# Glaciohound/Chimera-ST

Hardware: AMD Instinct MI355X
Metric: train utterances/sec, MuST-C EN-DE s2t_transformer_m, 1/2/4/8 MI355X (higher is better)
Workload: dtype bf16

## Files before the change

chimera-st_amd/csrc/elementwise.hip:

```cpp
#include "cst_common.h"

namespace {

inline int ew_blocks(int64_t items) {
  int64_t b = cst_ceil_div(items, 256);
  return (int)(b < 1 ? 1 : (b > 4096 ? 4096 : b));
}

template <typename T>
__global__ void glu_fwd_kernel(const T* z, T* y, int64_t rows, int64_t C) {
  const int64_t cv = C / 8, total = rows * cv;
  for (int64_t i = (int64_t)blockIdx.x * blockDim.x + threadIdx.x; i < total; i += (int64_t)gridDim.x * blockDim.x) {
    const int64_t r = i / cv, c = (i % cv) * 8;
    float a[8], g[8], o[8];
    load8(z + r * 2 * C + c, a);
    load8(z + r * 2 * C + C + c, g);
#pragma unroll
    for (int e = 0; e < 8; ++e) o[e] = a[e] / (1.0f + __expf(-g[e]));
    store8(y + r * C + c, o);
  }
}

template <typename T>
__global__ void glu_bwd_kernel(const T* dy, const T* z, T* dz, int64_t rows, int64_t C) {
// ... 531 lines not shown
    hipLaunchKernelGGL(wn_apply_fwd_kernel<bf16_t>, dim3(blocks), dim3(256), 0, s, (const bf16_t*)v, (const bf16_t*)g, (bf16_t*)w, norm, (const float*)workspace, nch, R, (int)C);
  } else {
    hipLaunchKernelGGL((wn_partial_kernel<float, false>), dim3(nch), dim3(256), 0, s, (const float*)v, (const float*)nullptr, (float*)workspace, R, (int)C);
    hipLaunchKernelGGL(wn_apply_fwd_kernel<float>, dim3(blocks), dim3(256), 0, s, (const float*)v, (const float*)g, (float*)w, norm, (const float*)workspace, nch, R, (int)C);
  }
  return cst_check_launch("cst_weight_norm_fwd");
}

extern "C" int cst_weight_norm_bwd(const void* v, const void* g, const void* dw, const float* norm, void* dv, void* dg, void* workspace, int64_t R,
                                   int64_t C, int dtype, cst_stream stream) {
  CST_REQUIRE(v && g && dw && norm && dv && dg && workspace && R > 0, "cst_weight_norm_bwd: null tensor");
  CST_REQUIRE(C % 8 == 0 && C >= 8 && C <= 256 && 256 % (C / 8) == 0, "cst_weight_norm_bwd: C = %lld", (long long)C);
  hipStream_t s = (hipStream_t)stream;
  CstProfScope prof(CST_K_ELEMENTWISE, s, 0.0, (double)R * C * cst_dtype_size(dtype) * 5);
  const int nch = (int)cst_ceil_div(R, WN_ROWS);
  const int blocks = (int)(cst_ceil_div(R * (C / 8), 256) < 1024 ? cst_ceil_div(R * (C / 8), 256) : 1024);
  if (dtype == CST_BF16) {
    hipLaunchKernelGGL((wn_partial_kernel<bf16_t, true>), dim3(nch), dim3(256), 0, s, (const bf16_t*)v, (const bf16_t*)dw, (float*)workspace, R, (int)C);
    hipLaunchKernelGGL(wn_apply_bwd_kernel<bf16_t>, dim3(blocks), dim3(256), 0, s, (const bf16_t*)v, (const bf16_t*)g, (const bf16_t*)dw, norm, (bf16_t*)dv, (bf16_t*)dg,
                       (const float*)workspace, nch, R, (int)C);
  } else {
    hipLaunchKernelGGL((wn_partial_kernel<float, true>), dim3(nch), dim3(256), 0, s, (const float*)v, (const float*)dw, (float*)workspace, R, (int)C);
    hipLaunchKernelGGL(wn_apply_bwd_kernel<float>, dim3(blocks), dim3(256), 0, s, (const float*)v, (const float*)g, (const float*)dw, norm, (float*)dv, (float*)dg,
                       (const float*)workspace, nch, R, (int)C);
  }
  return cst_check_launch("cst_weight_norm_bwd");
}

namespace {
template <typename T>
__device__ __forceinline__ void transpose_tile(const T* src, T* dst, int64_t R, int64_t C, int64_t r0, int64_t c0, T* tile) {
  constexpr int V = DT<T>::VEC, TS = 64, LDT = TS + V;
  constexpr int VPR = TS / V;
  for (int v = threadIdx.x; v < TS * VPR; v += 256) {
    const int r = v / VPR, cv = (v % VPR) * V;
    u32x4 x = {0, 0, 0, 0};
    if (r0 + r < R && c0 + cv < C) x = *reinterpret_cast<const u32x4*>(src + (r0 + r) * C + c0 + cv);
    *reinterpret_cast<u32x4*>(tile + r * LDT + cv) = x;
  }
  __syncthreads();
  for (int v = threadIdx.x; v < TS * VPR; v += 256) {
    const int c = v / VPR, rv = (v % VPR) * V;
    if (c0 + c < C && r0 + rv < R) {
      T out[V];
#pragma unroll
      for (int e = 0; e < V; ++e) out[e] = tile[(rv + e) * LDT + c];
      *reinterpret_cast<u32x4*>(dst + (c0 + c) * R + r0 + rv) = *reinterpret_cast<const u32x4*>(out);
    }
  }
}

template <typename T>
__global__ __launch_bounds__(256) void transpose2d_kernel(const T* src, T* dst, int64_t R, int64_t C) {
  __shared__ __attribute__((aligned(16))) T tile[64 * (64 + DT<T>::VEC)];
  transpose_tile<T>(src, dst, R, C, (int64_t)blockIdx.y * 64, (int64_t)blockIdx.x * 64, tile);
}

template <typename T>
__global__ __launch_bounds__(256) void transpose2d_multi_kernel(const cst_transpose_item* items, int n) {
  __shared__ __attribute__((aligned(16))) T tile[64 * (64 + DT<T>::VEC)];
  const int64_t b = blockIdx.x;
  int lo = 0, hi = n - 1;
  while (lo < hi) {
    const int mid = (lo + hi + 1) >> 1;
    if (items[mid].tile0 <= b) lo = mid; else hi = mid - 1;
  }
  const cst_transpose_item it = items[lo];
  const int64_t t = b - it.tile0, tx = (it.C + 63) / 64;
  transpose_tile<T>((const T*)it.src, (T*)it.dst, it.R, it.C, (t / tx) * 64, (t % tx) * 64, tile);
}
}

extern "C" int cst_transpose2d_multi(const cst_transpose_item* items_dev, int n, int64_t total_tiles, int dtype, cst_stream stream) {
  CST_REQUIRE(items_dev && n > 0 && total_tiles > 0 && total_tiles < (1ll << 31), "cst_transpose2d_multi: bad table");
  CST_REQUIRE(dtype == CST_F32 || dtype == CST_BF16, "cst_transpose2d_multi: bad dtype");
  hipStream_t s = (hipStream_t)stream;
  CstProfScope prof(CST_K_ELEMENTWISE, s, 0.0, 2.0 * (double)total_tiles * 4096 * cst_dtype_size(dtype));
  if (dtype == CST_BF16) hipLaunchKernelGGL(transpose2d_multi_kernel<bf16_t>, dim3((unsigned)total_tiles), dim3(256), 0, s, items_dev, n);
  else hipLaunchKernelGGL(transpose2d_multi_kernel<float>, dim3((unsigned)total_tiles), dim3(256), 0, s, items_dev, n);
  return cst_check_launch("cst_transpose2d_multi");
}

namespace {
struct ReduceTable { cst_reduce_item it[CST_REDUCE_MAX_ITEMS]; int n; };

__global__ __launch_bounds__(1024) void reduce_multi_kernel(ReduceTable t) {
  __shared__ float ra[64][65];
  const int b = blockIdx.x;
  int lo = 0, hi = t.n - 1;
  while (lo < hi) {
    const int mid = (lo + hi + 1) >> 1;
    if (t.it[mid].block0 <= b) lo = mid; else hi = mid - 1;
  }
  const cst_reduce_item& it = t.it[lo];
  const int64_t blk = b - it.block0;
  if (it.order == 0) {
    const int64_t i0 = (blk * 1024 + threadIdx.x) * 8;
    if (i0 >= it.L) return;
    const float* src = it.src + i0;
    float v[8] = {0.0f, 0.0f, 0.0f, 0.0f, 0.0f, 0.0f, 0.0f, 0.0f};
    int sp = 0;
    for (; sp + 4 <= it.P; sp += 4) {
      f32x4 a[4][2];
#pragma unroll
      for (int u = 0; u < 4; ++u) {
        a[u][0] = *reinterpret_cast<const f32x4*>(src + (int64_t)(sp + u) * it.stride);
        a[u][1] = *reinterpret_cast<const f32x4*>(src + (int64_t)(sp + u) * it.stride + 4);
      }
#pragma unroll
      for (int u = 0; u < 4; ++u)
#pragma unroll
        for (int e = 0; e < 4; ++e) { v[e] += a[u][0][e]; v[4 + e] += a[u][1][e]; }
    }
    for (; sp < it.P; ++sp) {
      const f32x4 a0 = *reinterpret_cast<const f32x4*>(src + (int64_t)sp * it.stride), a1 = *reinterpret_cast<const f32x4*>(src + (int64_t)sp * it.stride + 4);
#pragma unroll
      for (int e = 0; e < 4; ++e) { v[e] += a0[e]; v[4 + e] += a1[e]; }
    }
    if (it.dst_dtype == CST_BF16) store8((bf16_t*)it.dst + i0, v);
    else store8((float*)it.dst + i0, v);
    return;
  }
  const int cl = threadIdx.x & 15, g = threadIdx.x >> 4;
  const int64_t c = blk * 64 + cl * 4;
  f32x4 a = {0.0f, 0.0f, 0.0f, 0.0f};
  if (c < it.L) {
    const float* src = it.src + c;
    int i = g;
    for (; i + 192 < it.P; i += 256) {
      const f32x4 v0 = *reinterpret_cast<const f32x4*>(src + (int64_t)i * it.stride), v1 = *reinterpret_cast<const f32x4*>(src + (int64_t)(i + 64) * it.stride);
      const f32x4 v2 = *reinterpret_cast<const f32x4*>(src + (int64_t)(i + 128) * it.stride), v3 = *reinterpret_cast<const f32x4*>(src + (int64_t)(i + 192) * it.stride);
#pragma unroll
      for (int e = 0; e < 4; ++e) a[e] = (((a[e] + v0[e]) + v1[e]) + v2[e]) + v3[e];
    }
    for (; i < it.P; i += 64) {
      const f32x4 v = *reinterpret_cast<const f32x4*>(src + (int64_t)i * it.stride);
#pragma unroll
      for (int e = 0; e < 4; ++e) a[e] += v[e];
    }
  }
#pragma unroll
  for (int e = 0; e < 4; ++e) ra[g][cl * 4 + e] = a[e];
  __syncthreads();
  if (threadIdx.x < 64) {
    const int64_t cc = blk * 64 + threadIdx.x;
    if (cc < it.L) {
      float t = ra[0][threadIdx.x];
#pragma unroll 8
      for (int k = 1; k < 64; ++k) t += ra[k][threadIdx.x];
      if (it.dst_dtype == CST_BF16) DT<bf16_t>::st((bf16_t*)it.dst + cc, t);
      else ((float*)it.dst)[cc] = t;
    }
  }
}
}

extern "C" int cst_reduce_multi(const cst_reduce_item* items, int n, cst_stream stream) {
  CST_REQUIRE(items && n > 0 && n <= CST_REDUCE_MAX_ITEMS, "cst_reduce_multi: 1..%d items per call", CST_REDUCE_MAX_ITEMS);
  ReduceTable t;
  int64_t blocks = 0;
  double bytes = 0.0;
  for (int i = 0; i < n; ++i) {
    const cst_reduce_item& it = items[i];
    CST_REQUIRE(it.src && it.dst && it.L > 0 && it.L % 8 == 0 && it.P > 0 && it.stride % 4 == 0 && ((uintptr_t)it.src % 16) == 0 && ((uintptr_t)it.dst % 16) == 0,
                "cst_reduce_multi: item %d: L, stride, alignment", i);
    CST_REQUIRE((it.dst_dtype == CST_F32 || it.dst_dtype == CST_BF16) && (it.order == 0 || it.order == 1), "cst_reduce_multi: item %d: bad dst_dtype / order", i);
// ... 25 lines not shown
```

chimera-st_amd/csrc/gemm.hip:

```cpp
#include "gemm_common.h"
#include <vector>
#include <stdlib.h>
#include <string.h>
#include <type_traits>

namespace {
using namespace cstg;

template <int BM_, int BN_, int WM_, int WN_, int KV_ = 8>
struct Cfg {
  static constexpr int BM = BM_, BN = BN_, WM = WM_, WN = WN_, NT = 64 * WM_ * WN_, TM = BM_ / WM_ / 32, TN = BN_ / WN_ / 32;
  static constexpr int KV = KV_;
  static_assert(BM_ <= GEMM_MAX_BM && GEMM_MAX_BM % BM_ == 0, "conv0.hip (cst_conv_row_limits) sizes live frames from GEMM_MAX_BM");
};
using CfgSmall = Cfg<128, 128, 2, 2>;
using CfgSkinny = Cfg<64, 64, 2, 2>;
using CfgNarrowN = Cfg<128, 64, 2, 2>;
using CfgNarrowM = Cfg<64, 128, 2, 2>;
using CfgLarge = Cfg<256, 256, 4, 4>;

template <typename T, bool A_KMAJOR, bool B_KMAJOR, bool SEG, typename C, bool CS = false>
__global__ __launch_bounds__(C::NT) void gemm_kernel(GemmParams p) {
  constexpr int BM = C::BM, BN = C::BN, NTHREADS = C::NT, TM = C::TM, TN = C::TN;
  constexpr int VEC = DT<T>::VEC;
  constexpr int KV = C::KV, BK = KV * VEC;
  constexpr int LDK = BK + VEC;
  constexpr int LDMA = sizeof(T) == 2 ? BM + 32 : BM + VEC;
  constexpr int LDMB = sizeof(T) == 2 ? BN + 32 : BN + VEC;
  constexpr int A_ELEMS = A_KMAJOR ? BM * LDK : BK * LDMA;
  constexpr int B_ELEMS = B_KMAJOR ? BN * LDK : BK * LDMB;
  constexpr int MVA = BM / VEC, MVB = BN / VEC;
  constexpr int NVA = BM * KV / NTHREADS, NVB = BN * KV / NTHREADS;
  extern __shared__ __attribute__((aligned(16))) char smem_raw[];
  T* smem = reinterpret_cast<T*>(smem_raw);
  constexpr int STAGE = A_ELEMS + B_ELEMS;

  const int tid = threadIdx.x, lane = tid & 63, wave = tid >> 6;
  const int wm = wave / C::WN, wn = wave % C::WN;

  const int ntiles = p.tiles_m * p.tiles_n;
  int tm, tn, z;
  if (p.split_order) {
    const int total = ntiles * p.splits, L = (int)blockIdx.x + (int)gridDim.x * (int)blockIdx.z;
    const int q = total / 8, r = total % 8, xcd = L % 8, loc = L / 8;
    const int item = (xcd < r ? xcd * (q + 1) : r * (q + 1) + (xcd - r) * q) + loc;
    z = item / ntiles;
    const int t = item % ntiles;
    tm = t / p.tiles_n;
    tn = t % p.tiles_n;
  } else {
    int id = blockIdx.x;
    {
      const int q = ntiles / 8, r = ntiles % 8, xcd = id % 8, loc = id / 8;
      id = (xcd < r ? xcd * (q + 1) : r * (q + 1) + (xcd - r) * q) + loc;
    }
    constexpr int GROUP_M = 8;
    const int per_group = GROUP_M * p.tiles_n;
    const int grp = id / per_group, rem = id % per_group;
    const int gm0 = grp * GROUP_M;
    const int gsz = (p.tiles_m - gm0 < GROUP_M) ? (p.tiles_m - gm0) : GROUP_M;
    tm = gm0 + rem % gsz;
    tn = rem / gsz;
    z = blockIdx.z;
  }
  const int64_t m0 = (int64_t)tm * BM, n0 = (int64_t)tn * BN;

  const int split = z % p.splits;
  const int64_t bidx = z / p.splits;
  const int64_t b0 = bidx / p.batch1, b1 = bidx % p.batch1;
  const T* A = (const T*)p.A + b0 * p.sa0 + b1 * p.sa1;
  const T* B = (const T*)p.B + b0 * p.sb0 + b1 * p.sb1;
  const int64_t cofs = b0 * p.sc0 + b1 * p.sc1;
  const int64_t bofs = b0 * p.sbias0 + b1 * p.sbias1;

  int ktiles = (int)((p.K + BK - 1) / BK);
  const int kfull = (int)(p.K / BK);
  if (p.k_len) {
    typedef const __attribute__((address_space(4))) int32_t* cptr_t;
    const int kl = ((cptr_t)p.k_len)[b0];
    const int live = kl <= 0 ? 0 : (kl + BK - 1) / BK;
    ktiles = live < ktiles ? live : ktiles;
  }
  const int per = (ktiles + p.splits - 1) / p.splits;
  const int kt0 = split * per;
  const int kt1 = (kt0 + per < ktiles) ? kt0 + per : ktiles;

  u32x4 ra[NVA], rb[NVB];
  const T* pa[NVA];
  const T* pb[NVB];
  int ka[NVA], kb[NVB];
  int aq[NVA], ar[NVA], bq[NVB], br[NVB];
#pragma unroll
  for (int i = 0; i < NVA; ++i) {
    const int v = tid + NTHREADS * i;
    if (A_KMAJOR) {
      int64_t row = m0 + v / KV;
      row = row < p.M ? row : p.M - 1;
      ka[i] = kt0 * BK + (v % KV) * VEC;
      if (SEG && p.a_seg) { aq[i] = ka[i] / (int)p.a_seg; ar[i] = ka[i] % (int)p.a_seg; pa[i] = A + row * p.lda; }
      else { aq[i] = 0; ar[i] = 0; pa[i] = A + row * p.lda + ka[i]; }
    } else {
      int64_t m = m0 + (int64_t)(v % MVA) * VEC;
      m = m < p.M ? m : p.M - VEC;
      ka[i] = kt0 * BK + v / MVA;
      aq[i] = 0; ar[i] = 0;
      pa[i] = A + (int64_t)ka[i] * p.lda + segaddr(m, p.a_seg, p.a_seg_stride);
    }
  }
#pragma unroll
  for (int i = 0; i < NVB; ++i) {
    const int v = tid + NTHREADS * i;
    if (B_KMAJOR) {
      int64_t row = n0 + v / KV;
      row = row < p.N ? row : p.N - 1;
      kb[i] = kt0 * BK + (v % KV) * VEC;
      if (SEG && p.b_seg) { bq[i] = kb[i] / (int)p.b_seg; br[i] = kb[i] % (int)p.b_seg; pb[i] = B + row * p.ldb; }
      else { bq[i] = 0; br[i] = 0; pb[i] = B + row * p.ldb + kb[i]; }
    } else {
      int64_t n = n0 + (int64_t)(v % MVB) * VEC;
      n = n < p.N ? n : p.N - VEC;
      kb[i] = kt0 * BK + v / MVB;
      bq[i] = 0; br[i] = 0;
      pb[i] = B + (int64_t)kb[i] * p.ldb + segaddr(n, p.b_seg, p.b_seg_stride);
    }
  }
  const int64_t step_a = A_KMAJOR ? (int64_t)BK : (int64_t)BK * p.lda;
  const int64_t step_b = B_KMAJOR ? (int64_t)BK : (int64_t)BK * p.ldb;

  auto load_tile = [&](auto tail_tag) {
    constexpr bool TAIL = decltype(tail_tag)::value;
    const u32x4 zero = {0, 0, 0, 0};
#pragma unroll
    for (int i = 0; i < NVA; ++i) {
      const T* qa = pa[i];
      if (SEG && A_KMAJOR && p.a_seg) qa = pa[i] + (int64_t)aq[i] * p.a_seg_stride + ar[i];
      if (TAIL) {
        const bool oka = ka[i] < p.K;
        const u32x4 va = *reinterpret_cast<const u32x4*>(oka ? qa : A);
        ra[i] = oka ? va : zero;
      } else {
        ra[i] = *reinterpret_cast<const u32x4*>(qa);
      }
      ka[i] += BK;
      if (SEG && A_KMAJOR && p.a_seg) { ar[i] += BK; while (ar[i] >= (int)p.a_seg) { ar[i] -= (int)p.a_seg; ++aq[i]; } }
      else pa[i] += step_a;
    }
#pragma unroll
    for (int i = 0; i < NVB; ++i) {
      const T* qb = pb[i];
      if (SEG && B_KMAJOR && p.b_seg) qb = pb[i] + (int64_t)bq[i] * p.b_seg_stride + br[i];
      if (TAIL) {
        const bool okb = kb[i] < p.K;
        const u32x4 vb = *reinterpret_cast<const u32x4*>(okb ? qb : B);
        rb[i] = okb ? vb : zero;
      } else {
        rb[i] = *reinterpret_cast<const u32x4*>(qb);
      }
      kb[i] += BK;
      if (SEG && B_KMAJOR && p.b_seg) { br[i] += BK; while (br[i] >= (int)p.b_seg) { br[i] -= (int)p.b_seg; ++bq[i]; } }
      else pb[i] += step_b;
    }
  };
  auto load_any = [&](int kt) {
    if (kt < kfull) load_tile(std::false_type{});
    else load_tile(std::true_type{});
  };
  static_assert(!CS || (!A_KMAJOR && NTHREADS % MVA == 0), "a thread must stage the same columns of an mn-major A in every vector");
  const bool do_cs = CS && tn == 0;
  float cs[VEC];
#pragma unroll
  for (int e = 0; e < VEC; ++e) cs[e] = 0.0f;
  auto store_tile = [&](int buf) {
#pragma unroll
    for (int i = 0; i < NVA; ++i) {
      const int v = tid + NTHREADS * i;
      T* da = smem + buf * STAGE + (A_KMAJOR ? (v / KV) * LDK + (v % KV) * VEC : (v / MVA) * LDMA + (v % MVA) * VEC);
      *reinterpret_cast<u32x4*>(da) = ra[i];
      if (CS && do_cs) {
        if (sizeof(T) == 2) {
#pragma unroll
          for (int e = 0; e < 4; ++e) {
            cs[2 * e] += __uint_as_float(ra[i][e] << 16);
            cs[2 * e + 1] += __uint_as_float(ra[i][e] & 0xffff0000u);
          }
        } else {
#pragma unroll
          for (int e = 0; e < 4; ++e) cs[e] += __uint_as_float(ra[i][e]);
        }
      }
    }
#pragma unroll
    for (int i = 0; i < NVB; ++i) {
      const int v = tid + NTHREADS * i;
      T* db = smem + buf * STAGE + A_ELEMS + (B_KMAJOR ? (v / KV) * LDK + (v % KV) * VEC : (v / MVB) * LDMB + (v % MVB) * VEC);
      *reinterpret_cast<u32x4*>(db) = rb[i];
    }
  };

  f32x16 acc[TM][TN];
#pragma unroll
  for (int i = 0; i < TM; ++i)
#pragma unroll
    for (int j = 0; j < TN; ++j)
#pragma unroll
      for (int r = 0; r < 16; ++r) acc[i][j][r] = 0.0f;

  constexpr int KLIST_MAX = 1000;
  __shared__ int klist[KLIST_MAX];
  __shared__ int klist_n;
  const bool kskip = !SEG && BK == 64 && p.k_live != nullptr && per <= KLIST_MAX;
  int nk = kt1 > kt0 ? kt1 - kt0 : 0;
  if (kskip) {
    if (wave == 0) {
      int total = 0;
      for (int base = 0; base < ktiles; base += 64) {
        const int kt = base + lane;
        total += __builtin_popcountll(__builtin_amdgcn_ballot_w64(kt < ktiles && p.k_live[kt] == p.k_epoch));
      }
      const int lo = (int)(((int64_t)total * split) / p.splits), hi = (int)(((int64_t)total * (split + 1)) / p.splits);
      int seen = 0, n = 0;
      for (int base = 0; base < ktiles && seen < hi; base += 64) {
        const int kt = base + lane;
        const bool live = kt < ktiles && p.k_live[kt] == p.k_epoch;
        const uint64_t m = __builtin_amdgcn_ballot_w64(live);
        const int idx = seen + __builtin_popcountll(m & ((1ull << lane) - 1ull));
        if (live && idx >= lo && idx < hi) klist[idx - lo] = kt;
        seen += __builtin_popcountll(m);
      }
      n = hi - lo;
      if (lane == 0) klist_n = n;
    }
    __syncthreads();
    nk = klist_n;
  }
  if (p.m_live) {
    typedef const __attribute__((address_space(4))) uint32_t* cptr_t;
    cptr_t ml = (cptr_t)p.m_live;
    const int t0 = (int)(m0 >> 6), t1 = (int)((((m0 + BM < p.M) ? m0 + BM : p.M) + 63) >> 6);
    bool live = false;
    for (int t = t0; t < t1; ++t) live |= ml[t] == p.m_epoch;
    if (!live) nk = 0;
  }
  if (p.m_len) {
    typedef const __attribute__((address_space(4))) int32_t* cptr_t;
    if (m0 >= (int64_t)((cptr_t)p.m_len)[b0]) nk = 0;
  }
  int pos = kt0;
  auto fetch = [&](int kt) {
    const int d = kt - pos;
    if (d) {
#pragma unroll
      for (int i = 0; i < NVA; ++i) { pa[i] += (int64_t)d * step_a; ka[i] += d * BK; }
#pragma unroll
      for (int i = 0; i < NVB; ++i) { pb[i] += (int64_t)d * step_b; kb[i] += d * BK; }
    }
    load_any(kt);
    pos = kt + 1;
  };
  auto tile_at = [&](int it) { return kskip ? klist[it] : kt0 + it; };

  if (nk > 0) {
    fetch(tile_at(0));
    store_tile(0);
  }
  __syncthreads();
  int cur = 0;
  const int lrow = lane & 31, lk = 8 * (lane >> 5);
  constexpr int WROWS = TM * 32, WCOLS = TN * 32;
  for (int it = 0; it < nk; ++it) {
    const bool more = it + 1 < nk;
    if (more) fetch(tile_at(it + 1));
    const T* sa = smem + cur * STAGE;
    const T* sb = sa + A_ELEMS;
#pragma unroll
    for (int kk = 0; kk < BK; kk += 16) {
      Frag<T> fa[TM], fb[TN];
#pragma unroll
      for (int i = 0; i < TM; ++i) {
        if (A_KMAJOR) frag_load_contig(fa[i], sa + (wm * WROWS + i * 32 + lrow) * LDK + kk + lk);
        else frag_load_tr(fa[i], sa, LDMA, wm * WROWS + i * 32, kk + lk, kk + lk + 4, lane);
      }
#pragma unroll
      for (int j = 0; j < TN; ++j) {
        if (B_KMAJOR) frag_load_contig(fb[j], sb + (wn * WCOLS + j * 32 + lrow) * LDK + kk + lk);
        else frag_load_tr(fb[j], sb, LDMB, wn * WCOLS + j * 32, kk + lk, kk + lk + 4, lane);
      }
#pragma unroll
      for (int i = 0; i < TM; ++i)
#pragma unroll
        for (int j = 0; j < TN; ++j) mma16(acc[i][j], fa[i], fb[j]);
    }
    if (more) store_tile(cur ^ 1);
    __syncthreads();
    cur ^= 1;
  }

  if (CS && do_cs) {
    float* red = reinterpret_cast<float*>(smem_raw);
#pragma unroll
    for (int e = 0; e < VEC; ++e) red[(tid / MVA) * BM + (tid % MVA) * VEC + e] = cs[e];
    __syncthreads();
    if (tid < BM && m0 + tid < p.M) {
      float tot = 0.0f;
      for (int r = 0; r < NTHREADS / MVA; ++r) tot += red[r * BM + tid];
      if (p.splits > 1) p.colsum_ws[((int64_t)bidx * p.splits + split) * p.M + m0 + tid] = tot;
      else DT<T>::st((T*)p.colsum + bidx * p.M + m0 + tid, tot);
    }
  }

  constexpr int LDC = BN + 4;
  constexpr int VPR = BN / 8;
  constexpr int NPASS = BM / 64;
  constexpr int ITERS = 64 * VPR / NTHREADS;
  float* stage = reinterpret_cast<float*>(smem_raw);
  float* wsp = p.splits > 1 ? p.ws + ((int64_t)z) * p.M * p.N : nullptr;
  const bool ws_vec = (p.N % 4) == 0;
#pragma unroll
  for (int ps = 0; ps < NPASS; ++ps) {
    __syncthreads();
#pragma unroll
    for (int i = 0; i < TM; ++i) {
      const int trow = wm * WROWS + i * 32;
      if (trow / 64 == ps) {
#pragma unroll
        for (int j = 0; j < TN; ++j)
#pragma unroll
          for (int r = 0; r < 16; ++r)
            stage[(trow - 64 * ps + acc_row(r, lane)) * LDC + wn * WCOLS + j * 32 + lrow] = acc[i][j][r];
      }
    }
    __syncthreads();
#pragma unroll 2
    for (int it = 0; it < ITERS; ++it) {
      const int v = tid + NTHREADS * it;
      const int rl = v / VPR, cl = (v % VPR) * 8;
      const int64_t row = m0 + 64 * ps + rl, col = n0 + cl;
      if (row >= p.M || col >= p.N) continue;
      float x[8];
      {
        const f32x4 a = *reinterpret_cast<const f32x4*>(stage + rl * LDC + cl);
        const f32x4 b = *reinterpret_cast<const f32x4*>(stage + rl * LDC + cl + 4);
        x[0] = a[0]; x[1] = a[1]; x[2] = a[2]; x[3] = a[3]; x[4] = b[0]; x[5] = b[1]; x[6] = b[2]; x[7] = b[3];
      }
      const bool full = col + 8 <= p.N;
      if (wsp) {
        if (full && ws_vec) store8(wsp + row * p.N + col, x);
        else
          for (int e = 0; e < 8 && col + e < p.N; ++e) wsp[row * p.N + col + e] = x[e];
      } else if (full && p.vec_epi) {
        epilogue_store8<T>(p, cofs, bofs, row, col, x);
      } else {
        for (int e = 0; e < 8 && col + e < p.N; ++e) epilogue_store<T>(p, cofs, bofs, row, col + e, x[e]);
      }
    }
  }
}

template <int N>
__device__ __forceinline__ void wait_vmcnt() { asm volatile("s_waitcnt vmcnt(%0)" ::"n"(N) : "memory"); }

template <typename T, bool A_KMAJOR, bool B_KMAJOR, typename C, int NS>
__global__ __launch_bounds__(C::NT) void gemm_glds_kernel(GemmParams p) {
  constexpr int BM = C::BM, BN = C::BN, NTHREADS = C::NT, TM = C::TM, TN = C::TN, NWAVES = C::NT / 64;
  constexpr int ES = sizeof(T), VEC = DT<T>::VEC, BK = 128 / ES;
  constexpr int A_BYTES = A_KMAJOR ? BM * 128 : BK * BM * ES;
  constexpr int B_BYTES = B_KMAJOR ? BN * 128 : BK * BN * ES;
  constexpr int STAGE_BYTES = A_BYTES + B_BYTES;
  constexpr int GA = A_BYTES / 1024 / NWAVES, GB = B_BYTES / 1024 / NWAVES;
  extern __shared__ __attribute__((aligned(16))) char smem_raw[];

  const int tid = threadIdx.x, lane = tid & 63, wave = tid >> 6;
  const int wm = wave / C::WN, wn = wave % C::WN;
  const int ntiles = p.tiles_m * p.tiles_n;
  int id = blockIdx.x;
  {
    const int q = ntiles / 8, r = ntiles % 8, xcd = id % 8, loc = id / 8;
    id = (xcd < r ? xcd * (q + 1) : r * (q + 1) + (xcd - r) * q) + loc;
  }
  constexpr int GROUP_M = 8;
  int tm, tn;
  {
    const int per_group = GROUP_M * p.tiles_n;
    const int grp = id / per_group, rem = id % per_group;
    const int gm0 = grp * GROUP_M;
    const int gsz = (p.tiles_m - gm0 < GROUP_M) ? (p.tiles_m - gm0) : GROUP_M;
    tm = gm0 + rem % gsz;
    tn = rem / gsz;
  }
  const int64_t m0 = (int64_t)tm * BM, n0 = (int64_t)tn * BN;
  const int z = blockIdx.z;
  const int split = z % p.splits;
  const int64_t bidx = z / p.splits;
  const int64_t b0 = bidx / p.batch1, b1 = bidx % p.batch1;
  const T* A = (const T*)p.A + b0 * p.sa0 + b1 * p.sa1;
  const T* B = (const T*)p.B + b0 * p.sb0 + b1 * p.sb1;
  const int64_t cofs = b0 * p.sc0 + b1 * p.sc1;
  const int64_t bofs = b0 * p.sbias0 + b1 * p.sbias1;
  const int ktiles = (int)((p.K + BK - 1) / BK);
  const int kfull = (int)(p.K / BK);
  const int per = (ktiles + p.splits - 1) / p.splits;
  const int kt0 = split * per;
  const int kt1 = (kt0 + per < ktiles) ? kt0 + per : ktiles;
  int nt = kt1 - kt0;
  if (p.m_len) {
    typedef const __attribute__((address_space(4))) int32_t* cptr_t;
    if (m0 >= (int64_t)((cptr_t)p.m_len)[b0]) nt = 0;
  }

  const T* pa[GA];
  const T* pb[GB];
  int ka[GA], kb[GB];
#pragma unroll
  for (int i = 0; i < GA; ++i) {
    const int g = wave + NWAVES * i;
    if (A_KMAJOR) {
      const int r = 8 * g + (lane >> 3), c = (lane & 7) ^ ((r >> 1) & 7);
      int64_t row = m0 + r;
      row = row < p.M ? row : p.M - 1;
      ka[i] = kt0 * BK + c * VEC;
      pa[i] = A + row * p.lda + ka[i];
// ... 334 lines not shown
  p.tiles_m = (int)cst_ceil_div(M, C::BM);
  p.tiles_n = (int)cst_ceil_div(N, C::BN);
  p.split_order = (p.splits > 1 && nbatch == 1) ? 1 : 0;
  dim3 grid(p.tiles_m * p.tiles_n, 1, (unsigned)(nbatch * p.splits));
  if constexpr (!AK && !BK_ && !SEG && C::NT <= 256) {
    if (p.colsum) {
      static bool attr_cs = false;
      if (!attr_cs) {
        (void)hipFuncSetAttribute(reinterpret_cast<const void*>(&gemm_kernel<T, AK, BK_, SEG, C, true>), hipFuncAttributeMaxDynamicSharedMemorySize, 160 * 1024 - 4096);
        attr_cs = true;
      }
      hipLaunchKernelGGL((gemm_kernel<T, AK, BK_, SEG, C, true>), grid, dim3(C::NT), lds, s, p);
      return cst_check_launch("cst_gemm");
    }
  }
  if (p.colsum) { cst_set_error("cst_gemm: internal: column sums requested from a configuration that does not build them"); return CST_ERR_UNSUPPORTED; }
  hipLaunchKernelGGL((gemm_kernel<T, AK, BK_, SEG, C>), grid, dim3(C::NT), lds, s, p);
  return cst_check_launch("cst_gemm");
}

template <typename T, bool AK, bool BK_, typename C, int NS>
int launch_glds(GemmParams p, int64_t M, int64_t N, int64_t nbatch, hipStream_t s) {
  constexpr int ES = sizeof(T), BKc = 128 / ES;
  constexpr int A_BYTES = AK ? C::BM * 128 : BKc * C::BM * ES, B_BYTES = BK_ ? C::BN * 128 : BKc * C::BN * ES;
  size_t lds = (size_t)NS * (A_BYTES + B_BYTES);
  const size_t stage_bytes = (size_t)64 * (C::BN + 4) * sizeof(float);
  if (lds < stage_bytes) lds = stage_bytes;
  static bool attr_set = false;
  if (!attr_set) {
    (void)hipFuncSetAttribute(reinterpret_cast<const void*>(&gemm_glds_kernel<T, AK, BK_, C, NS>), hipFuncAttributeMaxDynamicSharedMemorySize, 160 * 1024);
    attr_set = true;
  }
  p.tiles_m = (int)cst_ceil_div(M, C::BM);
  p.tiles_n = (int)cst_ceil_div(N, C::BN);
  dim3 grid(p.tiles_m * p.tiles_n, 1, (unsigned)(nbatch * p.splits));
  hipLaunchKernelGGL((gemm_glds_kernel<T, AK, BK_, C, NS>), grid, dim3(C::NT), lds, s, p);
  return cst_check_launch("cst_gemm");
}


struct GemmSwitches {
  bool no_klive;
  int group_m;
  bool no_narrow;
  bool no_4w;
  bool experiment;
  const char* force_cfg;
};

GemmSwitches gemm_switches() {
  static const GemmSwitches once = [] {
    GemmSwitches w;
    w.no_klive = getenv("CST_GEMM_NO_KLIVE") != nullptr;
    const char* gm = getenv("CST_GEMM8P_GROUP_M");
    w.group_m = gm && atoi(gm) > 0 ? atoi(gm) : 4;
    w.no_narrow = getenv("CST_GEMM_NO_NARROW") != nullptr;
    w.no_4w = getenv("CST_GEMM_NO_4W") != nullptr;
    w.experiment = getenv("CST_GEMM_EXPERIMENT") != nullptr;
    w.force_cfg = nullptr;
    return w;
  }();
  GemmSwitches w = once;
  if (w.experiment) {
    const char* f = getenv("CST_GEMM_FORCE_CFG");
    w.force_cfg = f && *f ? f : nullptr;
  }
  return w;
}

enum class Family { Reg, Dma, Persistent8, FourWave };
enum class Tile { Small, Large, Skinny, NarrowN, NarrowM, Big4, Big4N, Unknown };
enum class Colsum { None, Fused, Separate };
using CfgBig4 = Cfg<256, 256, 2, 2>;
using CfgBig4N = Cfg<256, 192, 2, 2>;

struct GemmRoute {
  Family family;
  Tile tile;
  bool bf16, ak, bk;
  bool seg;
  int stages;
  int splits;
  Colsum colsum;
};

struct TileDims { int bm, bn, nt; };
template <typename C> constexpr TileDims dims_of() { return {C::BM, C::BN, C::NT}; }
constexpr TileDims kTileDims[] = {dims_of<CfgSmall>(),   dims_of<CfgLarge>(), dims_of<CfgSkinny>(), dims_of<CfgNarrowN>(),
                                  dims_of<CfgNarrowM>(), dims_of<CfgBig4>(),  dims_of<CfgBig4N>(),  {0, 0, 0}};

bool use_large(const cst_gemm_desc* d, bool seg, int splits) {
  if (seg) return false;
  const int64_t tiles = cst_ceil_div(d->M, 256) * cst_ceil_div(d->N, 256) * d->batch0 * d->batch1 * splits;
  return d->M >= 256 && d->N >= 256 && tiles >= 200;
}

int choose_splits(const cst_gemm_desc* d) {
  if (d->split_k > 1) return d->split_k;
  if (d->split_k == 0 || d->split_k == 1) return 1;
  const int bk = d->dtype == CST_BF16 ? 64 : 32;
  const int64_t ktiles = cst_ceil_div(d->K, bk);
  const int64_t nb = d->batch0 * d->batch1;
  if (d->M >= 256 && d->N >= 256) {
    const int64_t tl = cst_ceil_div(d->M, 256) * cst_ceil_div(d->N, 256) * nb;
    if (tl >= 200) return 1;
    int64_t s = 256 / tl;
    if (s > ktiles / 16) s = ktiles / 16;
    if (s > 32) s = 32;
    if (s >= 1 && tl * s >= 200) return (int)s;
  }
  const int64_t tiles = cst_ceil_div(d->M, 128) * cst_ceil_div(d->N, 128) * nb;
  if (tiles >= 256 || ktiles < 16) return 1;
  const int64_t cap = ktiles / 8 < 32 ? ktiles / 8 : 32;
  int64_t s1 = 256 / tiles, s2 = 512 / tiles;
  if (s1 > cap) s1 = cap;
  if (s2 > cap) s2 = cap;
  if (s1 < 1) s1 = 1;
  if (s2 < 1) s2 = 1;
  const int64_t s = (2.0 / (double)s2 < 0.9 / (double)s1) ? s2 : s1;
  return (int)s;
}

struct Forced { const char* name; bool kk; Family family; Tile tile; int stages; };
const Forced kForced[] = {
    {"small", false, Family::Reg, Tile::Small, 0},     {"narrowm", false, Family::Reg, Tile::NarrowM, 0},
    {"narrown", false, Family::Reg, Tile::NarrowN, 0}, {"skinny", false, Family::Reg, Tile::Skinny, 0},
    {"large", false, Family::Reg, Tile::Large, 0},     {"big4r", false, Family::Reg, Tile::Big4, 0},
    {"skinny4", true, Family::Dma, Tile::Skinny, 4},   {"skinny2", true, Family::Dma, Tile::Skinny, 2},
    {"small2", true, Family::Dma, Tile::Small, 2},     {"small3", true, Family::Dma, Tile::Small, 3},
    {"big4", true, Family::Dma, Tile::Big4, 2},        {"big4n", true, Family::Dma, Tile::Big4N, 2},
    {"big4r", true, Family::Reg, Tile::Big4, 0},       {"large", true, Family::Reg, Tile::Large, 0},
    {"8p", true, Family::Persistent8, Tile::Large, 0}, {"4w", true, Family::FourWave, Tile::Big4N, 0},
};

GemmRoute gemm_route(const cst_gemm_desc* d, const GemmParams& p, const GemmSwitches& sw) {
  GemmRoute r;
  r.bf16 = d->dtype == CST_BF16;
  r.ak = d->a_kmajor != 0;
  r.bk = d->b_kmajor != 0;
  r.seg = (r.ak && d->a_seg) || (r.bk && d->b_seg);
  r.stages = 2;
  r.splits = choose_splits(d);
  const bool kk = r.ak && r.bk, mm = !r.ak && !r.bk;
  const bool large = use_large(d, r.seg, r.splits);
  const int64_t nbatch = d->batch0 * d->batch1;
  r.colsum = !d->colsum ? Colsum::None : (mm && !d->a_seg && !d->b_seg && !large) ? Colsum::Fused : Colsum::Separate;
  auto take = [&r](Family f, Tile t, int stages = 2) { r.family = f; r.tile = t; r.stages = stages; return r; };

  if (!sw.no_narrow && !r.seg && !large && kk && d->N <= 64 && d->M > 256) return take(Family::Dma, Tile::NarrowN);
  if (!sw.no_narrow && !r.seg && !large && mm && d->M <= 64 && d->N > 256) return take(Family::Reg, Tile::NarrowM);

  GemmParams q = p;
  q.splits = r.splits;
  const bool unsplit1 = !r.seg && nbatch == 1 && r.splits == 1;
  if (sw.force_cfg && r.bf16 && !r.seg && nbatch == 1 && (mm || (kk && r.splits == 1))) {
    for (const Forced& f : kForced) {
      if (f.kk != kk || strcmp(f.name, sw.force_cfg) != 0) continue;
      if (f.family == Family::Persistent8 && !cst_gemm8p_supported(q, r.ak, r.bk, nbatch)) break;
      if (f.family == Family::FourWave && !cst_gemm4w_supported(q, r.ak, r.bk, nbatch)) break;
      return take(f.family, f.tile, f.stages);
    }
    return take(Family::Reg, Tile::Unknown);
  }

  const bool mid8p = kk && unsplit1 && d->M >= 256 && d->N >= 256 && cst_ceil_div(d->M, 256) * cst_ceil_div(d->N, 256) >= 150;
  if (kk && unsplit1 && (d->M <= 256 || (!large && !mid8p && cst_ceil_div(d->M, 128) * cst_ceil_div(d->N, 128) < 256))) {
    const bool two_stage = d->M > 256 && cst_ceil_div(d->M, 64) * cst_ceil_div(d->N, 64) > 512;
    return take(Family::Dma, Tile::Skinny, two_stage ? 2 : 4);
  }
  if (r.bf16 && !r.seg && !d->colsum) {
    if (!sw.no_4w && cst_gemm4w_supported(q, r.ak, r.bk, nbatch)) return take(Family::FourWave, Tile::Big4N);
    if (r.ak && (!d->dact || (!d->resid && !d->aux_out)) && (large || mid8p) && cst_gemm8p_supported(q, r.ak, r.bk, nbatch))
      return take(Family::Persistent8, Tile::Large);
  }
  const Tile t = large ? Tile::Large : Tile::Small;
  if (r.seg) return take(Family::Reg, Tile::Small);
  return take(kk && !d->colsum ? Family::Dma : Family::Reg, t);
}

void route_text(const GemmRoute& r, char* out, int64_t n) {
  const TileDims t = kTileDims[(int)r.tile];
  const char* dt = r.bf16 ? "bf16" : "f32";
  const char a = r.ak ? 'k' : 'm', b = r.bk ? 'k' : 'm';
  switch (r.family) {
    case Family::Reg:
      snprintf(out, (size_t)n, "reg %s %c%c%s %dx%d nt%d%s split%d", dt, a, b, r.seg ? " seg" : "", t.bm, t.bn, t.nt,
               r.colsum == Colsum::Fused ? " colsum" : "", r.splits);
      break;
    case Family::Dma: snprintf(out, (size_t)n, "glds %s %c%c %dx%d nt%d ns%d split%d", dt, a, b, t.bm, t.bn, t.nt, r.stages, r.splits); break;
    case Family::Persistent8: snprintf(out, (size_t)n, "8p %c%c", a, b); break;
    case Family::FourWave: snprintf(out, (size_t)n, "4w"); break;
  }
}

}

extern "C" int64_t cst_colsum_workspace(int64_t rows, int64_t cols);
extern "C" int cst_colsum_typed(const void* x, int64_t ldx, void* out, void* workspace, int64_t rows, int64_t cols, int dtype, int out_dtype, cst_stream stream);
extern "C" int cst_colsum_typed_live(const void* x, int64_t ldx, void* out, void* workspace, int64_t rows, int64_t cols, int dtype, int out_dtype,
                                     const uint32_t* row_live, uint32_t epoch, cst_stream stream);

namespace {

int validate(const cst_gemm_desc* d) {
  CST_REQUIRE(d && d->A && d->B && d->C, "cst_gemm: null operand");
  CST_REQUIRE(d->dtype == CST_F32 || d->dtype == CST_BF16, "cst_gemm: bad dtype %d", d->dtype);
  CST_REQUIRE(d->c_dtype == d->dtype || d->c_dtype == CST_F32, "cst_gemm: c_dtype must be dtype or f32");
  CST_REQUIRE(d->M > 0 && d->N > 0 && d->K > 0, "cst_gemm: empty problem M=%lld N=%lld K=%lld", (long long)d->M,
              (long long)d->N, (long long)d->K);
  const int vec = d->dtype == CST_BF16 ? 8 : 4;
  if (d->a_kmajor) CST_REQUIRE(d->K % vec == 0 && d->lda % vec == 0, "cst_gemm: k-major A needs K,lda %% %d == 0 (K=%lld lda=%lld)", vec, (long long)d->K, (long long)d->lda);
  else CST_REQUIRE(d->M % vec == 0 && d->lda % vec == 0, "cst_gemm: mn-major A needs M,lda %% %d == 0 (M=%lld lda=%lld)", vec, (long long)d->M, (long long)d->lda);
  if (d->b_kmajor) CST_REQUIRE(d->K % vec == 0 && d->ldb % vec == 0, "cst_gemm: k-major B needs K,ldb %% %d == 0 (K=%lld ldb=%lld)", vec, (long long)d->K, (long long)d->ldb);
  else CST_REQUIRE(d->N % vec == 0 && d->ldb % vec == 0, "cst_gemm: mn-major B needs N,ldb %% %d == 0 (N=%lld ldb=%lld)", vec, (long long)d->N, (long long)d->ldb);
  CST_REQUIRE(d->a_seg % vec == 0 && d->b_seg % vec == 0 && d->a_seg_stride % vec == 0 && d->b_seg_stride % vec == 0,
              "cst_gemm: segment sizes must be multiples of %d", vec);
  CST_REQUIRE(((uintptr_t)d->A % 16 == 0) && ((uintptr_t)d->B % 16 == 0), "cst_gemm: A/B must be 16-byte aligned");
  CST_REQUIRE(d->sa0 % vec == 0 && d->sa1 % vec == 0 && d->sb0 % vec == 0 && d->sb1 % vec == 0, "cst_gemm: batch strides of A/B must be multiples of %d", vec);
  CST_REQUIRE(d->batch0 >= 1 && d->batch1 >= 1, "cst_gemm: batch counts must be >= 1");
  CST_REQUIRE(!d->dact || d->aux_in, "cst_gemm: dact needs aux_in");
  CST_REQUIRE(d->drop_p >= 0.0f && d->drop_p < 1.0f, "cst_gemm: drop_p must be in [0, 1)");
  CST_REQUIRE(d->drop_p == 0.0f || d->batch0 * d->batch1 == 1, "cst_gemm: fused dropout needs an unbatched problem");
  CST_REQUIRE(!d->colsum || (!d->a_kmajor && !d->a_seg), "cst_gemm: colsum needs an mn-major, unsegmented A");
  return CST_OK;
}

GemmParams fill_params(const cst_gemm_desc* d, const GemmSwitches& sw) {
  GemmParams p;
  p.M = d->M; p.N = d->N; p.K = d->K;
  p.A = d->A; p.lda = d->lda; p.a_seg = d->a_seg; p.a_seg_stride = d->a_seg_stride;
  p.B = d->B; p.ldb = d->ldb; p.b_seg = d->b_seg; p.b_seg_stride = d->b_seg_stride;
  p.C = d->C; p.ldc = d->ldc;
  p.bias = d->bias; p.bias_mode = d->bias ? d->bias_mode : CST_BIAS_NONE; p.sbias0 = d->sbias0; p.sbias1 = d->sbias1;
  p.act = d->act;
  p.aux_out = d->aux_out; p.ld_aux_out = d->ld_aux_out;
  p.dact = d->dact; p.aux_in = d->aux_in; p.ld_aux_in = d->ld_aux_in;
  p.resid = d->resid; p.ld_resid = d->ld_resid;
  p.alpha = d->alpha;
  p.drop_thr = d->drop_p > 0.0f ? cst_drop_thr16(d->drop_p) : 0u;
  p.drop_key = d->drop_key;
  p.drop_scale = d->drop_p > 0.0f ? 1.0f / (1.0f - d->drop_p) : 1.0f;
  p.drop_row0 = 0;
  p.batch1 = d->batch1;
  p.sa0 = d->sa0; p.sa1 = d->sa1; p.sb0 = d->sb0; p.sb1 = d->sb1; p.sc0 = d->sc0; p.sc1 = d->sc1;
  p.c_f32 = (d->c_dtype == CST_F32 && d->dtype != CST_F32) ? 1 : 0;
  {
    auto al16 = [](const void* q) { return q == nullptr || ((uintptr_t)q % 16) == 0; };
    bool ok = d->ldc % 8 == 0 && d->sc0 % 8 == 0 && d->sc1 % 8 == 0 && al16(d->C) && al16(d->bias) && al16(d->aux_out) && al16(d->aux_in) && al16(d->resid);
    if (d->bias && d->bias_mode == CST_BIAS_COL) ok = ok && d->sbias0 % 8 == 0 && d->sbias1 % 8 == 0;
    if (d->aux_out) ok = ok && d->ld_aux_out % 8 == 0;
    if (d->aux_in) ok = ok && d->ld_aux_in % 8 == 0;
    if (d->resid) ok = ok && d->ld_resid % 8 == 0;
    if (d->drop_p > 0.0f) ok = ok && (d->N % 2 == 0);
    p.vec_epi = ok ? 1 : 0;
  }
  p.tiles_m = p.tiles_n = 0;
  p.split_order = 0;
  p.sched = nullptr;
  p.gperm_full = 0;
  p.mrot = 0;
  p.k_live = sw.no_klive ? nullptr : d->k_live;
  p.k_epoch = d->k_epoch;
  p.m_live = sw.no_klive ? nullptr : d->m_live;
  p.m_epoch = d->m_epoch;
  p.k_len = sw.no_klive ? nullptr : d->k_len;
  p.m_len = sw.no_klive ? nullptr : d->m_len;
  p.group_m = sw.group_m;
  p.splits = 1;
  p.ws = nullptr;
  p.colsum = nullptr;
  p.colsum_ws = nullptr;
  return p;
}

int64_t route_workspace(const cst_gemm_desc* d, const GemmRoute& r) {
  const int64_t s = r.splits, nb = d->batch0 * d->batch1;
  int64_t bytes = s > 1 ? s * d->M * d->N * nb * (int64_t)sizeof(float) : 0;
  if (r.colsum == Colsum::Fused) bytes += s > 1 ? s * d->M * nb * (int64_t)sizeof(float) : 0;
  else if (r.colsum == Colsum::Separate) bytes += cst_colsum_workspace(d->K, d->M);
  return bytes;
}

int take_route(const cst_gemm_desc* d, const GemmSwitches& sw, GemmParams& p, GemmRoute& r) {
  r = gemm_route(d, p, sw);
  const int64_t nbatch = d->batch0 * d->batch1;
  CST_REQUIRE(r.colsum != Colsum::Separate || (nbatch == 1 && d->M % 8 == 0 && d->lda % 8 == 0),
              "cst_gemm: colsum of this configuration runs as a separate column sum: unbatched, M and lda multiples of 8");
  CST_REQUIRE(cst_ceil_div(d->M, 128) * cst_ceil_div(d->N, 128) < (1ll << 31) && nbatch * r.splits < 65536, "cst_gemm: grid too large");
  p.splits = r.splits;
  p.colsum = r.colsum == Colsum::Fused ? d->colsum : nullptr;
#ifdef CST_TRACE
  if (p.splits == 1 && d->workspace) p.ws = (float*)d->workspace;
#endif
  const int64_t need = route_workspace(d, r);
  if (need > 0 && (!d->workspace || d->workspace_bytes < need)) {
    if (r.splits > 1) cst_set_error("cst_gemm: split_k=%d needs %lld workspace bytes, got %lld", r.splits, (long long)need, (long long)d->workspace_bytes);
    else cst_set_error("cst_gemm: colsum needs %lld workspace bytes, got %lld", (long long)need, (long long)d->workspace_bytes);
    return CST_ERR_WORKSPACE;
  }
  if (r.splits > 1) {
    p.ws = (float*)d->workspace;
    p.colsum_ws = p.ws + (int64_t)r.splits * d->M * d->N * nbatch;
  }
  return CST_OK;
}

template <typename W>
bool read_back(hipStream_t s, const W* dev, int64_t n, std::vector<W>& host) {
  host.resize((size_t)n);
  return hipStreamSynchronize(s) == hipSuccess && hipMemcpy(host.data(), dev, sizeof(W) * n, hipMemcpyDeviceToHost) == hipSuccess;
}

struct Work { double flops, bytes; };
Work credited_work(const cst_gemm_desc* d, const GemmParams& p, hipStream_t s) {
  double frac = 1.0;
  if (cst_prof_is_on()) {
    std::vector<uint32_t> st;
    std::vector<int32_t> len;
    const int64_t mtiles = cst_ceil_div(d->M, 256);
    if (p.k_live && read_back(s, p.k_live, cst_ceil_div(d->K, 64), st)) {
      int64_t live = 0;
      for (uint32_t v : st) live += v == p.k_epoch;
      frac *= (double)live / (double)st.size();
    }
    if (p.k_len && read_back(s, p.k_len, d->batch0, len)) {
      double sum = 0.0;
      for (int32_t v : len) sum += (double)(v < 0 ? 0 : (v < d->K ? v : d->K));
      frac *= sum / ((double)d->batch0 * (double)d->K);
    }
    if (p.m_len && read_back(s, p.m_len, d->batch0, len)) {
      double live = 0.0;
      for (int32_t v : len) {
        const int64_t t = v <= 0 ? 0 : cst_ceil_div((int64_t)v, 256);
        live += (double)(t < mtiles ? t : mtiles);
      }
      frac *= live / ((double)d->batch0 * (double)mtiles);
    }
    if (p.m_live && read_back(s, p.m_live, cst_ceil_div(d->M, 64), st)) {
      const int64_t nt = (int64_t)st.size();
      int64_t live = 0;
      for (int64_t t = 0; t < mtiles; ++t) {
        bool l = false;
        for (int64_t i = 4 * t; i < 4 * t + 4 && i < nt; ++i) l |= st[i] == p.m_epoch;
        live += l;
      }
      frac *= (double)live / (double)mtiles;
    }
  }
  const double nbatch = (double)(d->batch0 * d->batch1), esz = (double)cst_dtype_size(d->dtype);
  return {2.0 * (double)d->M * (double)d->N * (double)d->K * nbatch * frac,
          ((double)d->M * d->K + (double)d->N * d->K) * esz * nbatch * frac + (double)d->M * d->N * cst_dtype_size(d->c_dtype) * nbatch};
}

int unlaunchable(const GemmRoute& r, const GemmSwitches& sw) {
  if (r.tile == Tile::Unknown) {
    cst_set_error("cst_gemm: unknown CST_GEMM_FORCE_CFG %s", sw.force_cfg ? sw.force_cfg : "");
    return CST_ERR_BAD_ARG;
  }
  if (r.family == Family::Reg && r.colsum == Colsum::Fused && kTileDims[(int)r.tile].nt > 256) {
    cst_set_error("cst_gemm: internal: column sums requested from a configuration that does not build them");
    return CST_ERR_UNSUPPORTED;
  }
  return CST_OK;
}

template <typename T, bool SEG, typename C>
int launch_reg(const GemmRoute& r, const GemmParams& p, int64_t nbatch, hipStream_t s) {
  return r.ak ? (r.bk ? launch<T, true, true, SEG, C>(p, p.M, p.N, nbatch, s) : launch<T, true, false, SEG, C>(p, p.M, p.N, nbatch, s))
// ... 10 lines not shown
    case arm(Family::Persistent8, Tile::Large): return cst_gemm8p_launch(p, r.ak, r.bk, nbatch, s);
    case arm(Family::FourWave, Tile::Big4N): return cst_gemm4w_launch(p, s);
    case arm(Family::Reg, Tile::Small): return r.seg ? launch_reg<T, true, CfgSmall>(r, p, nbatch, s) : launch_reg<T, false, CfgSmall>(r, p, nbatch, s);
    case arm(Family::Reg, Tile::Large): return launch_reg<T, false, CfgLarge>(r, p, nbatch, s);
    case arm(Family::Reg, Tile::NarrowM): return launch<T, false, false, false, CfgNarrowM>(p, M, N, nbatch, s);
    case arm(Family::Dma, Tile::Small, 2): return launch_glds<T, true, true, CfgSmall, 2>(p, M, N, nbatch, s);
    case arm(Family::Dma, Tile::Large, 2): return launch_glds<T, true, true, CfgLarge, 2>(p, M, N, nbatch, s);
    case arm(Family::Dma, Tile::NarrowN, 2): return launch_glds<T, true, true, CfgNarrowN, 2>(p, M, N, nbatch, s);
    case arm(Family::Dma, Tile::Skinny, 2): return launch_glds<T, true, true, CfgSkinny, 2>(p, M, N, nbatch, s);
    case arm(Family::Dma, Tile::Skinny, 4): return launch_glds<T, true, true, CfgSkinny, 4>(p, M, N, nbatch, s);
    case arm(Family::Reg, Tile::NarrowN): if constexpr (HOOK) return launch<T, false, false, false, CfgNarrowN>(p, M, N, nbatch, s); break;
    case arm(Family::Reg, Tile::Skinny): if constexpr (HOOK) return launch<T, false, false, false, CfgSkinny>(p, M, N, nbatch, s); break;
    case arm(Family::Reg, Tile::Big4):
      if constexpr (HOOK) return r.ak ? launch<T, true, true, false, CfgBig4>(p, M, N, nbatch, s) : launch<T, false, false, false, CfgBig4>(p, M, N, nbatch, s);
      break;
    case arm(Family::Dma, Tile::Small, 3): if constexpr (HOOK) return launch_glds<T, true, true, CfgSmall, 3>(p, M, N, nbatch, s); break;
    case arm(Family::Dma, Tile::Big4, 2): if constexpr (HOOK) return launch_glds<T, true, true, CfgBig4, 2>(p, M, N, nbatch, s); break;
    case arm(Family::Dma, Tile::Big4N, 2): if constexpr (HOOK) return launch_glds<T, true, true, CfgBig4N, 2>(p, M, N, nbatch, s); break;
    default: break;
  }
  const int rc = unlaunchable(r, sw);
  if (rc == CST_OK) cst_set_error("cst_gemm: internal: a route without a launch arm");
  return rc == CST_OK ? CST_ERR_UNSUPPORTED : rc;
}

int finish(const cst_gemm_desc* d, const GemmRoute& r, const GemmParams& p, cst_stream stream) {
  const int64_t nbatch = d->batch0 * d->batch1;
  if (p.splits > 1 && d->defer_reduce) {
    CST_REQUIRE((nbatch == 1 || !d->colsum) && d->alpha == 1.0f && !d->bias && !d->act && !d->dact && !d->aux_out && !d->resid && d->drop_p == 0.0f && d->ldc == d->N &&
                    d->N % 8 == 0 && r.colsum != Colsum::Separate,
                "cst_gemm: defer_reduce needs a plain epilogue and a dense C (batched: no colsum; the slabs are [batch][split][M][N])");
    return CST_OK;
  }
  int rc = CST_OK;
  if (p.splits > 1) {
    const int64_t total = d->M * d->N;
    const int64_t work = (p.vec_epi && d->N % 8 == 0) ? total / 8 : total;
    int blocks = (int)(cst_ceil_div(work, 256) < 2048 ? cst_ceil_div(work, 256) : 2048);
    dim3 grid(blocks, (unsigned)nbatch);
    if (d->dtype == CST_BF16) hipLaunchKernelGGL(splitk_reduce_kernel<bf16_t>, grid, dim3(256), 0, (hipStream_t)stream, p);
    else hipLaunchKernelGGL(splitk_reduce_kernel<float>, grid, dim3(256), 0, (hipStream_t)stream, p);
    rc = cst_check_launch("cst_gemm split-k reduce");
  }
  if (rc == CST_OK && r.colsum == Colsum::Separate) {
    void* cws = (char*)d->workspace + (p.splits > 1 ? (int64_t)p.splits * d->M * d->N * (int64_t)sizeof(float) : 0);
    rc = p.k_live ? cst_colsum_typed_live(d->A, d->lda, d->colsum, cws, d->K, d->M, d->dtype, d->dtype, p.k_live, p.k_epoch, stream)
                  : cst_colsum_typed(d->A, d->lda, d->colsum, cws, d->K, d->M, d->dtype, d->dtype, stream);
  }
  return rc;
}

int gemm_one(const cst_gemm_desc* d, cst_stream stream) {
  int rc = validate(d);
  if (rc != CST_OK) return rc;
  const GemmSwitches sw = gemm_switches();
  GemmParams p = fill_params(d, sw);
  GemmRoute r;
  if ((rc = take_route(d, sw, p, r)) != CST_OK) return rc;
  hipStream_t s = (hipStream_t)stream;
  const int64_t nbatch = d->batch0 * d->batch1;
  const Work w = credited_work(d, p, s);
  CstProfScope prof(CST_K_GEMM, s, w.flops, w.bytes);
  rc = r.bf16 ? launch_route<bf16_t>(r, p, nbatch, s, sw) : launch_route<float>(r, p, nbatch, s, sw);
  if (cst_prof_is_on())
    prof.tag("M=%lld N=%lld K=%lld b=%lld a%c b%c split=%d%s%s%s%s%s%s%s", (long long)d->M, (long long)d->N, (long long)d->K, (long long)nbatch, r.ak ? 'k' : 'm',
             r.bk ? 'k' : 'm', p.splits, d->bias ? " bias" : "", d->act ? " act" : "", d->aux_out ? " aux_out" : "", d->dact ? " dact" : "",
             d->resid ? " resid" : "", d->drop_p > 0 ? " drop" : "", (d->k_live || d->m_live || d->k_len || d->m_len) ? " live" : "");
  return rc != CST_OK ? rc : finish(d, r, p, stream);
}

GemmRoute query_route(const cst_gemm_desc* d) {
  const GemmSwitches sw = gemm_switches();
  return gemm_route(d, fill_params(d, sw), sw);
}

}

extern "C" int cst_gemm_splits(const cst_gemm_desc* d) { return d ? query_route(d).splits : 0; }

extern "C" int cst_gemm_colsum_is_fused(const cst_gemm_desc* d) { return d && query_route(d).colsum == Colsum::Fused ? 1 : 0; }

extern "C" int64_t cst_gemm_workspace(const cst_gemm_desc* d) { return route_workspace(d, query_route(d)); }

extern "C" int cst_gemm_route(const cst_gemm_desc* d, char* out, int64_t out_bytes) {
  if (out && out_bytes > 0) out[0] = 0;
  int rc = validate(d);
  if (rc != CST_OK) return rc;
  CST_REQUIRE(out && out_bytes > 0, "cst_gemm_route: no room for the text");
  const GemmSwitches sw = gemm_switches();
  GemmParams p = fill_params(d, sw);
  GemmRoute r;
  if ((rc = take_route(d, sw, p, r)) != CST_OK) return rc;
  if ((rc = unlaunchable(r, sw)) != CST_OK) return rc;
  route_text(r, out, out_bytes);
  return CST_OK;
}

extern "C" int cst_gemm(const cst_gemm_desc* d, cst_stream stream) { return gemm_one(d, stream); }
```

chimera-st_amd/csrc/gemm8p.hip:

```cpp
#include "gemm_common.h"
#include <atomic>
#include <cstdlib>
#include <mutex>
#include <type_traits>

namespace {
using namespace cstg;
using T = bf16_t;

constexpr int BM = 256, BN = 256, BK = 64, NTHREADS = 512;
static_assert(BM <= cstg::GEMM_MAX_BM && cstg::GEMM_MAX_BM % BM == 0, "conv0.hip (cst_conv_row_limits) sizes live frames from GEMM_MAX_BM");
constexpr int QB = 17408;
constexpr int GSTRIDE = 1088;
constexpr int KSTRIDE = 1024;
constexpr int BUFB = 4 * QB;
constexpr int LDS_BYTES = 2 * BUFB;
constexpr unsigned OOB = 0x80000000u;

template <int N>
__device__ __forceinline__ void wait_vm() { asm volatile("s_waitcnt vmcnt(%0)" ::"n"(N) : "memory"); }
template <int N>
__device__ __forceinline__ void wait_lgkm() { asm volatile("s_waitcnt lgkmcnt(%0)" ::"n"(N) : "memory"); }

__device__ __forceinline__ unsigned lds_off(const void* p) {
// ... 29 lines not shown
  const int wave = __builtin_amdgcn_readfirstlane(tid >> 6);
  const int wm = wave >> 2, wn = wave & 3;
  const int lrow = lane & 31, hi = lane >> 5;
  const int ntiles = p.tiles_m * p.tiles_n;
  const int total = p.nitems;
  const int ktiles = (int)((p.K + BK - 1) / BK);
  const int per = (ktiles + p.splits - 1) / p.splits;
  typedef const __attribute__((address_space(4))) GemmParams* kparg_t;
  kparg_t kp = (kparg_t)__builtin_amdgcn_kernarg_segment_ptr();

  const int ck = (lane & 7) ^ (((4 * wave) + (lane >> 4)) & 7);
  const int klm = 16 * (wave >> 2) + 4 * (lane >> 4) + (wave & 3);
  const int kla = AK ? ck * 8 : klm, klb = BKM ? ck * 8 : klm;
  const int pa = AK ? 8 * wave + (lane >> 3) : (lane & 15) * 8;
  const int pb = BKM ? 8 * wave + (lane >> 3) : (lane & 15) * 8;
  const unsigned step_a = AK ? (unsigned)(BK * 2) : (unsigned)(BK * p.lda * 2);
  const unsigned step_b = BKM ? (unsigned)(BK * 2) : (unsigned)(BK * p.ldb * 2);
  constexpr bool EXF = MODE == 2;
  const bool fast_epi = MODE != 0 || (!p.c_f32 && p.splits == 1 && p.vec_epi && (p.N % 8) == 0 && p.bias_mode != CST_BIAS_ROW &&
                                (p.bias_mode == CST_BIAS_NONE || p.alpha == 1.0f));
  const bool bias_in_acc = fast_epi && p.bias_mode == CST_BIAS_COL;
  char* const bias_lds = smem + 2 * BUFB;

  __amdgpu_buffer_rsrc_t ra, rb;
  unsigned va0 = 0, vb0 = 0;
  int nt = 0, krem0 = 0, mrem = 0, nrem = 0;
  int hf = 0;
  unsigned lda2 = 0, ldb2 = 0;
  int64_t m0 = 0, n0 = 0, cofs = 0, bofs = 0;
  int zcur = 0;

  auto setup = [&](int v) {
    asm volatile("" : "+s"(kp));
    struct { int64_t M, N, K, lda, ldb, batch1, sa0, sa1, sb0, sb1, sc0, sc1, sbias0, sbias1; const void *A, *B, *bias; int splits, tiles_m, tiles_n; } p;
    p.M = kp->M; p.N = kp->N; p.K = kp->K; p.lda = kp->lda; p.ldb = kp->ldb; p.batch1 = kp->batch1;
    p.sa0 = kp->sa0; p.sa1 = kp->sa1; p.sb0 = kp->sb0; p.sb1 = kp->sb1; p.sc0 = kp->sc0; p.sc1 = kp->sc1;
    p.sbias0 = kp->sbias0; p.sbias1 = kp->sbias1; p.A = kp->A; p.B = kp->B; p.bias = kp->bias;
    p.splits = kp->splits; p.tiles_m = kp->tiles_m; p.tiles_n = kp->tiles_n;
    auto fdiv = [](int n, unsigned long long magic) { return (int)(((unsigned long long)(unsigned)n * magic) >> 40); };
    int half = -1, vt = v;
    if (v >= kp->half_from) {
      const int o = v - kp->half_from;
      half = o & 1;
      vt = kp->half_from + (o >> 1);
    }
    hf = half >= 0 ? 1 : 0;
    const int z = kp->nz > 1 ? fdiv(vt, kp->magic_ntiles) : 0;
    int id = vt - z * ntiles;
    {
      const int q = ntiles >> 3, r = ntiles & 7, xcd = id & 7, loc = id >> 3;
      id = (xcd < r ? xcd * (q + 1) : r * (q + 1) + (xcd - r) * q) + loc;
    }
    if (kp->mrot > 0) {
      int zr = z * kp->mrot;
      zr -= fdiv(zr, kp->magic_ntiles) * ntiles;
      id += zr;
      if (id >= ntiles) id -= ntiles;
    }
    const int GROUP_M = kp->group_m, per_group = kp->per_group, gshift = kp->group_shift;
    int grp = fdiv(id, kp->magic_per_group);
    const int rem = id - grp * per_group;
    if (kp->gperm_full > 0 && grp < kp->gperm_full) {
      const int q = kp->gperm_q, r = kp->gperm_r, big = (q + 1) * r;
      int col, row;
      if (grp < big) { col = fdiv(grp, kp->magic_gq1); row = grp - col * (q + 1); }
      else { const int t = grp - big, c = fdiv(t, kp->magic_gq); col = r + c; row = t - c * q; }
      grp = row * 8 + col;
    }
    const int gm0 = grp * GROUP_M;
    const int gsz = (p.tiles_m - gm0 < GROUP_M) ? (p.tiles_m - gm0) : GROUP_M;
    int tm, tn;
    if (gsz == GROUP_M && gshift >= 0) { tm = gm0 + (rem & (GROUP_M - 1)); tn = rem >> gshift; }
    else { tm = gm0 + rem % gsz; tn = rem / gsz; }
    m0 = (int64_t)tm * BM + (half == 1 ? 128 : 0);
    n0 = (int64_t)tn * BN;
    zcur = z;
    const int split = p.splits > 1 ? z % p.splits : 0;
    const int64_t bidx = p.splits > 1 ? z / p.splits : z;
    const int64_t b0 = p.batch1 > 1 ? bidx / p.batch1 : bidx, b1 = p.batch1 > 1 ? bidx % p.batch1 : 0;
    const T* A = (const T*)p.A + b0 * p.sa0 + b1 * p.sa1;
    const T* B = (const T*)p.B + b0 * p.sb0 + b1 * p.sb1;
    cofs = b0 * p.sc0 + b1 * p.sc1;
    bofs = b0 * p.sbias0 + b1 * p.sbias1;
    const int kt0 = split * per;
    const int kt1 = (kt0 + per < ktiles) ? kt0 + per : ktiles;
    nt = kt1 > kt0 ? kt1 - kt0 : 0;
    if (kp->m_live) {
      typedef const __attribute__((address_space(4))) uint32_t* cptr_t;
      cptr_t ml = (cptr_t)kp->m_live;
      const uint32_t ep = kp->m_epoch;
      const int t0 = (int)(m0 >> 6), tn = (int)((p.M + 63) >> 6);
      bool live = false;
#pragma unroll
      for (int i = 0; i < 4; ++i) live |= (i < 2 || !hf) && (t0 + i < tn) && ml[t0 + i < tn ? t0 + i : t0] == ep;
      if (!live) nt = 0;
    }
    if (kp->m_len) {
      typedef const __attribute__((address_space(4))) int32_t* iptr_t;
      if (m0 >= (int64_t)((iptr_t)kp->m_len)[b0]) nt = 0;
    }
    krem0 = (int)p.K - kt0 * BK;
    const T* abase = AK ? A + m0 * p.lda + (int64_t)kt0 * BK : A + (int64_t)kt0 * BK * p.lda + m0;
    const T* bbase = BKM ? B + n0 * p.ldb + (int64_t)kt0 * BK : B + (int64_t)kt0 * BK * p.ldb + n0;
    ra = __builtin_amdgcn_make_buffer_rsrc((void*)abase, (short)0, (int)OOB, 0x00020000);
    rb = __builtin_amdgcn_make_buffer_rsrc((void*)bbase, (short)0, (int)OOB, 0x00020000);
    if (bias_in_acc) {
      const int64_t left = p.N - n0;
      const __amdgpu_buffer_rsrc_t rbias = __builtin_amdgcn_make_buffer_rsrc((void*)((const T*)p.bias + bofs + n0), (short)0,
                                                                              (int)((left < 256 ? left : 256) * 2), 0x00020000);
      dma16(rbias, bias_lds, (unsigned)lane * 16);
    }
    lda2 = (unsigned)(p.lda * 2);
    ldb2 = (unsigned)(p.ldb * 2);
    mrem = (int)(p.M - m0 < BM ? p.M - m0 : BM);
    if (hf && mrem > 128) mrem = 128;
    if (mrem <= 0) { mrem = 0; nt = 0; }
    nrem = (int)(p.N - n0 < BN ? p.N - n0 : BN);
    va0 = AK ? (unsigned)pa * lda2 + (unsigned)kla * 2 : (unsigned)klm * lda2 + (unsigned)pa * 2;
    vb0 = BKM ? (unsigned)pb * ldb2 + (unsigned)klb * 2 : (unsigned)klm * ldb2 + (unsigned)pb * 2;
  };

  auto stage = [&](auto qc, auto bufc, int tau) {
    constexpr int Q = decltype(qc)::value, BUF = decltype(bufc)::value;
    constexpr bool IS_A = (Q & 1) != 0;
    constexpr int H = Q >> 1;
    constexpr bool KM = IS_A ? AK : BKM;
    constexpr int GS = KM ? KSTRIDE : GSTRIDE;
    const int krem = krem0 - tau * BK;
    const unsigned ld2 = IS_A ? lda2 : ldb2;
    const unsigned base = (IS_A ? va0 : vb0) + (unsigned)tau * (IS_A ? step_a : step_b) + (KM ? (unsigned)(H * 128) * ld2 : (unsigned)(H * 256));
    const int pos = (IS_A ? pa : pb) + H * 128;
    const int lim = IS_A ? mrem : nrem;
    char* dst = smem + BUF * BUFB + Q * QB + wave * GS;
#pragma unroll
    for (int j = 0; j < 2; ++j) {
      const unsigned v0 = base + (KM ? (unsigned)(64 * j) * ld2 : (unsigned)(32 * j) * ld2);
      const bool ok = ((IS_A ? kla : klb) + (KM ? 0 : 32 * j) < krem) && (pos + (KM ? 64 * j : 0) < lim);
      dma16(IS_A ? ra : rb, dst + j * 8 * GS, ok ? v0 : OOB);
    }
  };
  using I0 = std::integral_constant<int, 0>;
  using I1 = std::integral_constant<int, 1>;
  using I2 = std::integral_constant<int, 2>;
  using I3 = std::integral_constant<int, 3>;

  const int swr = (lrow >> 1) & 7;
  const int arow = (wm * 64 + lrow) * 128, brow = (wn * 32 + lrow) * 128;
  const int trl = ((lane & 15) >> 2) * GSTRIDE + hi * 512 + (16 * ((lane >> 4) & 1) + 4 * (lane & 3)) * 2;
  auto read_tr = [&](Frag<T>& f, const char* q) {
    const v4s_t x = __builtin_amdgcn_ds_read_tr16_b64_v4i16((v4s_t __attribute__((address_space(3)))*)(q));
    const v4s_t y = __builtin_amdgcn_ds_read_tr16_b64_v4i16((v4s_t __attribute__((address_space(3)))*)(q + 256));
    u16x8 t;
    t[0] = (unsigned short)x[0]; t[1] = (unsigned short)x[1]; t[2] = (unsigned short)x[2]; t[3] = (unsigned short)x[3];
    t[4] = (unsigned short)y[0]; t[5] = (unsigned short)y[1]; t[6] = (unsigned short)y[2]; t[7] = (unsigned short)y[3];
    f.v = __builtin_bit_cast(bf16x8, t);
  };
  auto read_a = [&](Frag<T>& f, const char* img, int i, int kk) {
    if (AK) f.v = *reinterpret_cast<const bf16x8*>(img + arow + i * 4096 + (((2 * kk + hi) ^ swr) << 4));
    else read_tr(f, img + trl + wm * 128 + i * 64 + kk * 4 * GSTRIDE);
  };
  auto read_b = [&](Frag<T>& f, const char* img, int kk) {
    if (BKM) f.v = *reinterpret_cast<const bf16x8*>(img + brow + (((2 * kk + hi) ^ swr) << 4));
    else read_tr(f, img + trl + wn * 64 + kk * 4 * GSTRIDE);
  };

  f32x16 acc[4][2];
  Frag<T> fa[2][4], fb0[4], fb1[4];

  auto mfma_quadrant = [&](auto hmc, auto hnc) {
    constexpr int HM = decltype(hmc)::value, HN = decltype(hnc)::value;
    __builtin_amdgcn_s_setprio(1);
#pragma unroll
    for (int kk = 0; kk < 4; ++kk)
#pragma unroll
      for (int i = 0; i < 2; ++i) mma16(acc[HM * 2 + i][HN], HN ? fb1[kk] : fb0[kk], fa[i][kk]);
    __builtin_amdgcn_s_setprio(0);
  };

  auto tile_body = [&](auto bufc, int t, int S, const bool half) {
    constexpr int BUF = decltype(bufc)::value;
    using BC = std::integral_constant<int, BUF>;
    using BN_ = std::integral_constant<int, BUF ^ 1>;
    const char* img = smem + BUF * BUFB;
    const int s0 = 7 + 4 * t;
#pragma unroll
    for (int kk = 0; kk < 4; ++kk) read_b(fb0[kk], img + 0 * QB, kk);
    __builtin_amdgcn_sched_barrier(0);
#pragma unroll
    for (int kk = 0; kk < 4; ++kk)
#pragma unroll
      for (int i = 0; i < 2; ++i) read_a(fa[i][kk], img + 1 * QB, i, kk);
    __builtin_amdgcn_sched_barrier(0);
    if (s0 < S) stage(I3{}, BN_{}, t + 1);
    wait_lgkm<AK ? 8 : 15>();
    __builtin_amdgcn_s_barrier();
    wait_lgkm<0>();
    __builtin_amdgcn_sched_barrier(0);
// ... 54 lines not shown
    const int S = 4 * nt;
    if (0 < S) stage(I0{}, I0{}, 0);
    if (1 < S) stage(I1{}, I0{}, 0);
    if (2 < S) stage(I2{}, I0{}, 0);
    if (3 < S) stage(I3{}, I0{}, 0);
  }
  claim_issue();
  claim_land();
#ifdef CST_TRACE
  long long* trace = (p.splits == 1 && p.ws) ? reinterpret_cast<long long*>(p.ws) + (int64_t)blockIdx.x * 64 : nullptr;
  int titem = 0;
#define CST_STAMP(k) do { if (trace && tid == 0 && titem < 8) trace[titem * 8 + (k)] = (long long)__builtin_readcyclecounter(); } while (0)
#else
#define CST_STAMP(k) do { } while (0)
#endif
  while (true) {
    CST_STAMP(0);
    const int64_t e_m0 = m0, e_n0 = n0, e_cofs = cofs, e_bofs = bofs;
    const int e_z = zcur, e_nt = nt;
    const bool e_hf = hf != 0;
    const int S = 4 * e_nt;
    if (4 < S) stage(I0{}, I1{}, 1);
    if (5 < S) stage(I1{}, I1{}, 1);
    if (6 < S) stage(I2{}, I1{}, 1);
    if (7 <= S) wait_vm<6>();
    else wait_vm<0>();
    __builtin_amdgcn_s_barrier();
    if (bias_in_acc) {
#pragma unroll
      for (int hn = 0; hn < 2; ++hn)
#pragma unroll
        for (int g = 0; g < 4; ++g) {
          const uint2 raw = *reinterpret_cast<const uint2*>(bias_lds + (hn * 128 + wn * 32 + 8 * g + 4 * hi) * 2);
          const float b0 = __uint_as_float(raw.x << 16), b1 = __uint_as_float(raw.x & 0xffff0000u);
          const float b2 = __uint_as_float(raw.y << 16), b3 = __uint_as_float(raw.y & 0xffff0000u);
#pragma unroll
          for (int i = 0; i < 4; ++i) {
            acc[i][hn][4 * g] = b0; acc[i][hn][4 * g + 1] = b1; acc[i][hn][4 * g + 2] = b2; acc[i][hn][4 * g + 3] = b3;
          }
        }
      wait_lgkm<0>();
    } else {
#pragma unroll
      for (int i = 0; i < 4; ++i)
#pragma unroll
        for (int j = 0; j < 2; ++j)
#pragma unroll
          for (int r = 0; r < 16; ++r) acc[i][j][r] = 0.0f;
    }
    if (wm == 1) __builtin_amdgcn_s_barrier();
    CST_STAMP(1);
    for (int t = 0; t < e_nt; t += 2) {
      tile_body(I0{}, t, S, e_hf);
      if (t + 1 < e_nt) tile_body(I1{}, t + 1, S, e_hf);
    }
    if (wm == 0) __builtin_amdgcn_s_barrier();
    CST_STAMP(2);

    {
      int item;
      asm volatile("ds_read_b32 %0, %1\n\ts_waitcnt lgkmcnt(0)" : "=v"(item) : "v"(slot_off + 4u * (unsigned)par) : "memory");
      v = __builtin_amdgcn_readfirstlane(p.sched ? item : v + (int)gridDim.x);
    }
    const bool has_next = v < total;
    if (has_next) {
      claim_issue();
      setup(v);
      CST_STAMP(5);
      const int Sn = 4 * nt;
      if (0 < Sn) stage(I0{}, I0{}, 0);
      if (1 < Sn) stage(I1{}, I0{}, 0);
      if (2 < Sn) stage(I2{}, I0{}, 0);
      if (3 < Sn) stage(I3{}, I0{}, 0);
      CST_STAMP(6);
    }

    CST_STAMP(3);
    asm volatile("" : "+s"(kp));
    GemmParams q;
    q.M = kp->M; q.N = kp->N; q.C = kp->C; q.ldc = kp->ldc; q.bias = kp->bias; q.bias_mode = kp->bias_mode; q.act = kp->act;
    q.aux_out = kp->aux_out; q.ld_aux_out = kp->ld_aux_out; q.dact = kp->dact; q.aux_in = kp->aux_in; q.ld_aux_in = kp->ld_aux_in;
    q.resid = kp->resid; q.ld_resid = kp->ld_resid; q.alpha = kp->alpha; q.splits = kp->splits; q.ws = kp->ws;
    q.c_f32 = kp->c_f32; q.vec_epi = kp->vec_epi; q.drop_thr = kp->drop_thr; q.drop_key = kp->drop_key; q.drop_scale = kp->drop_scale; q.drop_row0 = kp->drop_row0;
    if (fast_epi && e_nt == 0 && q.bias_mode == CST_BIAS_NONE && !q.resid) {
      if (has_next) claim_land();
      const u32x4 z4 = {0u, 0u, 0u, 0u};
      const int64_t col = e_n0 + (tid & 31) * 8;
      if (col < q.N) {
        T* const cb = (T*)q.C + e_cofs + col;
        T* const xb = q.aux_out ? (T*)q.aux_out + e_cofs + col : nullptr;
#pragma unroll 4
        for (int it = 0; it < (e_hf ? 8 : 16); ++it) {
          const int64_t row = e_m0 + (tid >> 5) + 16 * it;
          if (row < q.M) {
            __builtin_nontemporal_store(z4, reinterpret_cast<u32x4*>(cb + row * q.ldc));
            if (xb) __builtin_nontemporal_store(z4, reinterpret_cast<u32x4*>(xb + row * q.ld_aux_out));
          }
        }
      }
    } else if (fast_epi) {
      constexpr int ERS = 528;
      const T* exsrc = MODE == 1 ? nullptr : (q.dact ? (const T*)q.aux_in : (const T*)q.resid);
      const int64_t exld = q.dact ? q.ld_aux_in : q.ld_resid;
      const bool both = q.dact && q.resid;
      constexpr bool ex_fast = EXF;
      u32x4 exq[8];
      const T* ex_b = nullptr;
      if (ex_fast) {
        int64_t colc = e_n0 + (tid & 31) * 8;
        colc = colc < q.N ? colc : q.N - 8;
        ex_b = exsrc + e_cofs + colc;
#pragma unroll
        for (int it = 0; it < 8; ++it) {
          int64_t row = e_m0 + (tid >> 5) + 16 * it;
          row = row < q.M ? row : q.M - 1;
          exq[it] = __builtin_nontemporal_load(reinterpret_cast<const u32x4*>(ex_b + row * exld));
        }
      }
#pragma unroll
      for (int hm = 0; hm < 2; ++hm) {
        if (hm && e_hf) break;
        if (hm) __builtin_amdgcn_s_barrier();
#pragma unroll
        for (int i = 0; i < 2; ++i)
#pragma unroll
          for (int hn = 0; hn < 2; ++hn)
#pragma unroll
            for (int g = 0; g < 4; ++g) {
              typedef __bf16 bf16x4_t __attribute__((ext_vector_type(4)));
              bf16x4_t pk;
#pragma unroll
              for (int e = 0; e < 4; ++e) pk[e] = static_cast<__bf16>(acc[hm * 2 + i][hn][4 * g + e] * q.alpha);
              lds_write_b64(ebase_off + (wm * 64 + i * 32 + lrow) * ERS + (hn * 128 + wn * 32 + 8 * g + 4 * hi) * 2, __builtin_bit_cast(uint2, pk));
            }
        wait_lgkm<0>();
        __builtin_amdgcn_s_barrier();
        if (hm == 0 && has_next) claim_land();
        if (exsrc && !ex_fast) {
#pragma unroll 2
          for (int it = 0; it < 8; ++it) {
            const int vi = tid + NTHREADS * it;
            const int rl = vi >> 5, cl = (vi & 31) * 8;
            const int64_t row = e_m0 + hm * 128 + rl, col = e_n0 + cl;
            if (row >= q.M || col >= q.N) continue;
            const u32x4 exv = *reinterpret_cast<const u32x4*>(exsrc + e_cofs + row * exld + col);
            const u32x4 zraw = lds_read_b128(ebase_off + rl * ERS + cl * 2);
            wait_lgkm<0>();
            __builtin_amdgcn_sched_barrier(0);
            if (q.aux_out) *reinterpret_cast<u32x4*>((T*)q.aux_out + e_cofs + row * q.ld_aux_out + col) = zraw;
            float x[8];
#pragma unroll
            for (int e = 0; e < 4; ++e) {
              x[2 * e] = __uint_as_float(zraw[e] << 16);
              x[2 * e + 1] = __uint_as_float(zraw[e] & 0xffff0000u);
            }
            if (q.act == CST_ACT_RELU) {
#pragma unroll
              for (int e = 0; e < 8; ++e) x[e] = fmaxf(x[e], 0.0f);
            } else if (q.act == CST_ACT_GELU) {
#pragma unroll
              for (int e = 0; e < 8; ++e) x[e] = gelu_t<T>(x[e]);
            }
            if (q.drop_thr) cst_drop8(x, q.drop_key, (uint64_t)((row + q.drop_row0) * q.N + col), q.drop_thr, q.drop_scale);
            if (q.dact) {
#pragma unroll
              for (int e = 0; e < 4; ++e) {
// ... 157 lines not shown
          if (row >= q.M || col >= q.N) continue;
          float x[8];
          {
            const u32x4 ua = lds_read_b128(ebase_off + (rl * LDC + cl) * 4), ub = lds_read_b128(ebase_off + (rl * LDC + cl + 4) * 4);
            wait_lgkm<0>();
            __builtin_amdgcn_sched_barrier(0);
            const f32x4 a = __builtin_bit_cast(f32x4, ua), b = __builtin_bit_cast(f32x4, ub);
            x[0] = a[0]; x[1] = a[1]; x[2] = a[2]; x[3] = a[3]; x[4] = b[0]; x[5] = b[1]; x[6] = b[2]; x[7] = b[3];
          }
          const bool full = col + 8 <= q.N;
          if (wsp) {
            if (full && ws_vec) store8(wsp + row * q.N + col, x);
            else
              for (int e = 0; e < 8 && col + e < q.N; ++e) wsp[row * q.N + col + e] = x[e];
          } else if (full && q.vec_epi) {
            epilogue_store8<T>(q, e_cofs, e_bofs, row, col, x);
          } else {
            for (int e = 0; e < 8 && col + e < q.N; ++e) epilogue_store<T>(q, e_cofs, e_bofs, row, col + e, x[e]);
          }
        }
      }
    }
    CST_STAMP(4);
#ifdef CST_TRACE
    ++titem;
#endif
    if (!has_next) break;
    __builtin_amdgcn_s_barrier();
  }
  int* const sched_exit = p.sched;
  if (int* const sched = sched_exit; sched && tid == 0) {
    if (atomicAdd(sched + 8, 1) == (int)gridDim.x - 1) {
#pragma unroll
      for (int i = 0; i < 9; ++i) __hip_atomic_store(sched + i, 0, __ATOMIC_RELAXED, __HIP_MEMORY_SCOPE_AGENT);
    }
  }
}

int* sched_slot() {
  constexpr int SLOTS = 1024, MAXDEV = 64;
  static int* ring[MAXDEV] = {};
  static std::atomic<unsigned> next[MAXDEV];
  static std::mutex mu;
  int dev = 0;
  if (hipGetDevice(&dev) != hipSuccess || dev < 0 || dev >= MAXDEV) return nullptr;
  int* r = __atomic_load_n(&ring[dev], __ATOMIC_ACQUIRE);
  if (!r) {
    std::lock_guard<std::mutex> g(mu);
    r = ring[dev];
    if (!r) {
      void* q = nullptr;
      if (hipMalloc(&q, SLOTS * 64) != hipSuccess) return nullptr;
      if (hipMemset(q, 0, SLOTS * 64) != hipSuccess || hipDeviceSynchronize() != hipSuccess) return nullptr;
      r = (int*)q;
      __atomic_store_n(&ring[dev], r, __ATOMIC_RELEASE);
    }
  }
  return r + 16 * (next[dev].fetch_add(1, std::memory_order_relaxed) % SLOTS);
}

std::atomic<int> g_reserved_cus{[] { const char* e = getenv("CST_GEMM_RESERVE_CUS"); return e ? atoi(e) : 0; }()};

template <bool AK, bool BKM, int MODE>
int launch8p(GemmParams p, int64_t nbatch, hipStream_t s) {
  static bool attr_set = false;
  if (!attr_set) {
    (void)hipFuncSetAttribute(reinterpret_cast<const void*>(&gemm8p_kernel<AK, BKM, MODE>), hipFuncAttributeMaxDynamicSharedMemorySize, 160 * 1024);
    attr_set = true;
  }
  p.tiles_m = (int)cst_ceil_div(p.M, BM);
  p.tiles_n = (int)cst_ceil_div(p.N, BN);
  p.nz = (int)(nbatch * p.splits);
  const int64_t total = (int64_t)p.tiles_m * p.tiles_n * p.nz;
  {
    const int64_t ntl = (int64_t)p.tiles_m * p.tiles_n;
    p.per_group = p.group_m * p.tiles_n;
    if (total * ntl >= (1ll << 40) || total * (int64_t)p.per_group >= (1ll << 40)) { cst_set_error("cst_gemm (8-phase): too many work items"); return CST_ERR_BAD_ARG; }
    p.magic_ntiles = ((1ull << 40) / (unsigned long long)ntl) + 1ull;
    p.magic_per_group = ((1ull << 40) / (unsigned long long)p.per_group) + 1ull;
    p.group_shift = -1;
    for (int sft = 0; sft < 16; ++sft)
      if ((1 << sft) == p.group_m) p.group_shift = sft;
    const int gfull = p.tiles_m / p.group_m;
    p.gperm_full = (p.m_len && gfull >= 16) ? gfull : 0;
    p.mrot = (p.m_len && p.gperm_full == 0 && ntl >= 2) ? (int)(ntl / 8 > 0 ? ntl / 8 : 1) : 0;
    p.gperm_q = gfull / 8;
    p.gperm_r = gfull % 8;
    p.magic_gq = p.gperm_q > 0 ? ((1ull << 40) / (unsigned long long)p.gperm_q) + 1ull : 0ull;
    p.magic_gq1 = ((1ull << 40) / (unsigned long long)(p.gperm_q + 1)) + 1ull;
  }
  static const int ncu = [] {
    int dev = 0, n = 256;
    (void)hipGetDevice(&dev);
    (void)hipDeviceGetAttribute(&n, hipDeviceAttributeMultiprocessorCount, dev);
    return n > 0 ? n : 256;
  }();
  const int avail = ncu - g_reserved_cus.load(std::memory_order_relaxed) > 8 ? ncu - g_reserved_cus.load(std::memory_order_relaxed) : 8;
  const bool no_halves = getenv("CST_GEMM8P_NO_HALVES") != nullptr;
  int64_t nitems = total;
  p.half_from = 0x7fffffff;
  if (!no_halves && p.nz == 1 && total > avail) {
    const int64_t r = total % avail;
    if (r > 0 && 2 * r <= avail) {
      p.half_from = (int)(total - r);
      nitems = total + r;
    }
  }
  p.nitems = (int)nitems;
  dim3 grid((unsigned)(nitems < avail ? nitems : avail), 1, 1);
  static const bool static_walk = getenv("CST_GEMM8P_STATIC") != nullptr;
  hipStreamCaptureStatus cap = hipStreamCaptureStatusNone;
  const bool capturing = hipStreamIsCapturing(s, &cap) != hipSuccess || cap != hipStreamCaptureStatusNone;
  p.sched = (!static_walk && !capturing && nitems > avail && grid.x % 8 == 0) ? sched_slot() : nullptr;
  hipLaunchKernelGGL((gemm8p_kernel<AK, BKM, MODE>), grid, dim3(NTHREADS), LDS_BYTES + 1024 + 64, s, p);
  return cst_check_launch("cst_gemm (8-phase)");
}

}

extern "C" int cst_gemm_reserve_cus(int n) {
  const int old = g_reserved_cus.load();
  if (n >= 0) g_reserved_cus.store(n > 248 ? 248 : n);
  return old;
}

bool cst_gemm8p_supported(const cstg::GemmParams& p, bool ak, bool bk, int64_t nbatch) {
  (void)nbatch;
  if (p.a_seg || p.b_seg) return false;
  const int64_t lim = (int64_t)1 << 31;
  const int64_t ea = ak ? (256 * p.lda + p.K) * 2 : (p.K + 64) * p.lda * 2;
  const int64_t eb = bk ? (256 * p.ldb + p.K) * 2 : (p.K + 64) * p.ldb * 2;
  return ea < lim && eb < lim && p.lda > 0 && p.ldb > 0;
}

int cst_gemm8p_launch(cstg::GemmParams p, bool ak, bool bk, int64_t nbatch, hipStream_t s) {
  const bool fast = !p.c_f32 && p.splits == 1 && p.vec_epi && (p.N % 8) == 0 && p.bias_mode != CST_BIAS_ROW &&
                    (p.bias_mode == CST_BIAS_NONE || p.alpha == 1.0f);
  const bool exf = fast && !p.aux_out && ((p.dact != 0) != (p.resid != nullptr)) && (!p.dact || p.aux_in);
  const bool plainf = fast && !p.dact && !p.resid;
#define CST_8P_MODE(MODE)                                                                                          \
  (ak ? (bk ? launch8p<true, true, MODE>(p, nbatch, s) : launch8p<true, false, MODE>(p, nbatch, s))              \
      : (bk ? launch8p<false, true, MODE>(p, nbatch, s) : launch8p<false, false, MODE>(p, nbatch, s)))
  if (exf) return CST_8P_MODE(2);
  if (plainf) return CST_8P_MODE(1);
  return CST_8P_MODE(0);
#undef CST_8P_MODE
}
```

chimera-st_amd/csrc/gemm_common.h:

```cpp
#pragma once
#include "cst_common.h"

namespace cstg {

constexpr int GEMM_MAX_BM = 256;

struct GemmParams {
  int64_t M, N, K;
  const void* A; int64_t lda, a_seg, a_seg_stride;
  const void* B; int64_t ldb, b_seg, b_seg_stride;
  void* C; int64_t ldc;
  const void* bias; int bias_mode; int64_t sbias0, sbias1;
  int act;
  void* aux_out; int64_t ld_aux_out;
  int dact;
  const void* aux_in; int64_t ld_aux_in;
  const void* resid; int64_t ld_resid;
  float alpha;
  uint32_t drop_thr, drop_key; float drop_scale;
  int64_t drop_row0;
  int64_t batch1;
  int64_t sa0, sa1, sb0, sb1, sc0, sc1;
  int splits;
  float* ws;
  int c_f32;
  int vec_epi;
  int tiles_m, tiles_n;
  int nz;
  int half_from, nitems;
  int group_m;
  unsigned long long magic_ntiles, magic_per_group;
  int per_group, group_shift;
  int gperm_full, gperm_q, gperm_r;
  int mrot;
  unsigned long long magic_gq, magic_gq1;
  int split_order;
  int* sched;
  const uint32_t* m_live; uint32_t m_epoch;
  const int32_t* k_len;
  const int32_t* m_len;
  const uint32_t* k_live; uint32_t k_epoch;
  void* colsum;
  float* colsum_ws;
};

__device__ __forceinline__ int64_t segaddr(int64_t c, int64_t seg, int64_t seg_stride) {
  return seg ? (c / seg) * seg_stride + (c % seg) : c;
}

template <typename T>
__device__ __forceinline__ void epilogue_store(const GemmParams& p, int64_t cofs, int64_t bofs, int64_t row, int64_t col, float v) {
  v *= p.alpha;
  if (p.bias_mode == CST_BIAS_COL) v += DT<T>::ld((const T*)p.bias + bofs + col);
  else if (p.bias_mode == CST_BIAS_ROW) v += DT<T>::ld((const T*)p.bias + bofs + row);
  if (p.aux_out) DT<T>::st((T*)p.aux_out + cofs + row * p.ld_aux_out + col, v);
  v = act_t<T>(v, p.act);
  if (p.drop_thr) v *= cst_drop1(p.drop_key, (uint64_t)((row + p.drop_row0) * p.N + col), p.drop_thr, p.drop_scale);
  if (p.dact) v *= dact_t<T>(DT<T>::ld((const T*)p.aux_in + cofs + row * p.ld_aux_in + col), p.dact);
  if (p.resid) v += DT<T>::ld((const T*)p.resid + cofs + row * p.ld_resid + col);
  if (p.c_f32) ((float*)p.C)[cofs + row * p.ldc + col] = v;
  else DT<T>::st((T*)p.C + cofs + row * p.ldc + col, v);
}

template <typename T>
__device__ __forceinline__ void epilogue_store8(const GemmParams& p, int64_t cofs, int64_t bofs, int64_t row, int64_t col, float (&v)[8]) {
#pragma unroll
  for (int e = 0; e < 8; ++e) v[e] *= p.alpha;
  if (p.bias_mode == CST_BIAS_COL) {
    float b[8];
    load8((const T*)p.bias + bofs + col, b);
#pragma unroll
    for (int e = 0; e < 8; ++e) v[e] += b[e];
  } else if (p.bias_mode == CST_BIAS_ROW) {
    const float b = DT<T>::ld((const T*)p.bias + bofs + row);
#pragma unroll
    for (int e = 0; e < 8; ++e) v[e] += b;
  }
  if (p.aux_out) store8((T*)p.aux_out + cofs + row * p.ld_aux_out + col, v);
  if (p.act == CST_ACT_RELU) {
#pragma unroll
    for (int e = 0; e < 8; ++e) v[e] = fmaxf(v[e], 0.0f);
  } else if (p.act == CST_ACT_GELU) {
#pragma unroll
    for (int e = 0; e < 8; ++e) v[e] = gelu_t<T>(v[e]);
  }
  if (p.drop_thr) cst_drop8(v, p.drop_key, (uint64_t)((row + p.drop_row0) * p.N + col), p.drop_thr, p.drop_scale);
  if (p.dact) {
    float z[8];
    load8((const T*)p.aux_in + cofs + row * p.ld_aux_in + col, z);
#pragma unroll
    for (int e = 0; e < 8; ++e) v[e] *= dact_t<T>(z[e], p.dact);
  }
  if (p.resid) {
    float r[8];
    load8((const T*)p.resid + cofs + row * p.ld_resid + col, r);
#pragma unroll
    for (int e = 0; e < 8; ++e) v[e] += r[e];
  }
  if (p.c_f32) store8((float*)p.C + cofs + row * p.ldc + col, v);
  else store8((T*)p.C + cofs + row * p.ldc + col, v);
}

}

int cst_gemm8p_launch(cstg::GemmParams p, bool a_kmajor, bool b_kmajor, int64_t nbatch, hipStream_t s);
bool cst_gemm8p_supported(const cstg::GemmParams& p, bool a_kmajor, bool b_kmajor, int64_t nbatch);
int cst_gemm4w_launch(cstg::GemmParams p, hipStream_t s);
bool cst_gemm4w_supported(const cstg::GemmParams& p, bool a_kmajor, bool b_kmajor, int64_t nbatch);
```

chimera-st_amd/functional.py:

```python
import os as _os
import weakref as _weakref

import torch

from . import kernels as K
from . import lib as L

_ACT = {None: L.ACT_NONE, "none": L.ACT_NONE, "relu": L.ACT_RELU, "gelu": L.ACT_GELU}


def _flat2d(x):
    return x.reshape(-1, x.shape[-1]).contiguous()


def _vec(dtype):
    return 8 if dtype == torch.bfloat16 else 4


def _with_tiles(t, tiles):
    if t.is_contiguous():
        t._cst_live_tiles = (tiles[0], tiles[1], t.data_ptr(), t.numel(), t.shape[-1], t._version)
        if t._base is not None:
            t._base._cst_live_tiles = t._cst_live_tiles
    return t
# ... 700 lines not shown


def ln_gelu(u, ln_weight, ln_bias, conv_bias=None, eps=1e-5, row_limit=None):
    return _LnGeluFn.apply(u, ln_weight, ln_bias, conv_bias, eps, row_limit)


def _padded_base(t, L, C):
    if t.dim() == 3 and t.stride(2) == 1 and t.stride(1) == C and t.stride(0) == (L + 2) * C and t.storage_offset() >= C:
        return torch.as_strided(t, (t.shape[0], L + 2, C), t.stride(), t.storage_offset() - C)
    return None


class _Conv1dCLFn(torch.autograd.Function):

    @staticmethod
    def forward(ctx, x, w_cl, bias, k, stride, pad, act, prev_z, grad_is_dz, nz_out=None, nz_in=None, unread_ok=False):
        if _os.environ.get("CST_NO_MLEN"):
            nz_in = None
            fwd_len = None
        else:
            fwd_len = nz_out if (bias is None or unread_ok) else None
        ctx.nz_out = nz_out
        ctx.nz_in = nz_in
        B, Lin, Cin = x.shape
        Cout = w_cl.shape[0]
        if pad:
            xp = torch.empty(B, Lin + 2 * pad, Cin, dtype=x.dtype, device=x.device)
            xp[:, :pad].zero_()
            xp[:, pad + Lin:].zero_()
            xp[:, pad:pad + Lin] = x
        elif x.stride(2) == 1 and x.stride(1) == Cin:
            xp = x
        else:
            xp = x.contiguous()
        Lp = Lin + 2 * pad
        Lout = (Lp - k) // stride + 1
        padded_out = bool(grad_is_dz) and act != L.ACT_NONE
        rows = Lout + 2 if padded_out else Lout
        y_full = torch.empty(B, rows, Cout, dtype=x.dtype, device=x.device)
        z_full = torch.empty_like(y_full) if act != L.ACT_NONE else None
        coff = Cout if padded_out else 0
        K.gemm(xp, w_cl, y_full, Lout, Cout, k * Cin, a_kmajor=1, b_kmajor=1, lda=stride * Cin, ldb=k * Cin, ldc=Cout, bias=bias,
               act=act, aux_out=z_full, ld_aux_out=Cout, batch0=B, sa=(xp.stride(0), 0), sc=(rows * Cout, 0), split_k=1,
               a_off=0, c_off=coff, m_len=fwd_len)
        y = y_full[:, 1:1 + Lout] if padded_out else y_full
        z = (z_full[:, 1:1 + Lout] if padded_out else z_full) if z_full is not None else None
        ctx.save_for_backward(xp, w_cl, z, prev_z)
        ctx.cfg = (B, Lin, Cin, Cout, k, stride, pad, Lout, act, bias is not None, grad_is_dz)
        ctx.set_materialize_grads(False)
        if act != L.ACT_NONE:
            ctx.mark_non_differentiable(z)
            return y, z
        return y, None

    @staticmethod
    def backward(ctx, dy, _dz_unused):
        xp, w_cl, z, prev_z = ctx.saved_tensors
        B, Lin, Cin, Cout, k, stride, pad, Lout, act, has_bias, grad_is_dz = ctx.cfg
        fast = pad == 0 and k <= stride + 1
        dzp = _padded_base(dy, Lout, Cout) if (act == L.ACT_NONE or grad_is_dz) else None
        if dzp is None:
            dyc = dy.contiguous()
            dzc = K.act_bwd(dyc, z.contiguous(), act) if (act != L.ACT_NONE and not grad_is_dz) else dyc
            if fast:
                dzp = torch.empty(B, Lout + 2, Cout, dtype=dy.dtype, device=dy.device)
                dzp[:, 0].zero_()
                dzp[:, Lout + 1].zero_()
                dzp[:, 1:1 + Lout] = dzc
            dz_rows, dz_bs, dz_off = dzc, Lout * Cout, 0
        else:
            dz_rows, dz_bs, dz_off = dzp, (Lout + 2) * Cout, Cout
        dx = dw = db = None
        if ctx.needs_input_grad[0]:
            if fast:
                dx_padded = prev_z is not None and _padded_base(prev_z, Lin, Cin) is not None
                rows = Lin + 2 if dx_padded else Lin
                dx_full = torch.empty(B, rows, Cin, dtype=dy.dtype, device=dy.device)
                if dx_padded:
                    dx_full[:, 0].zero_()
                    dx_full[:, Lin + 1].zero_()
                pz = prev_z if prev_z is None or dx_padded else prev_z.contiguous()
                pz_base = _padded_base(prev_z, Lin, Cin) if dx_padded else pz
                w3 = w_cl.view(Cout, k, Cin)
                for r in range(stride):
                    taps = list(range(r, k, stride))
                    n = len(taps)
                    U = (Lin - r + stride - 1) // stride
                    if n == 0 or U <= 0:
                        continue
                    wr = w3[:, r::stride, :].flip(1).permute(2, 1, 0).reshape(Cin, n * Cout).contiguous()
                    ml = ctx.nz_in[r] if ctx.nz_in is not None else None
                    K.gemm(dzp, wr, dx_full, U, Cin, n * Cout, a_kmajor=1, b_kmajor=1, lda=Cout, ldb=n * Cout, ldc=stride * Cin,
                           batch0=B, sa=((Lout + 2) * Cout, 0), sc=(rows * Cin, 0), a_off=(2 - n) * Cout,
                           c_off=(Cin if dx_padded else 0) + r * Cin, dact=L.ACT_GELU if prev_z is not None else L.ACT_NONE,
                           aux_in=pz_base, ld_aux_in=stride * Cin, split_k=1, m_len=ml)
                dx = dx_full[:, 1:1 + Lin] if dx_padded else dx_full
            else:
                dz2 = dz_rows.reshape(B * Lout, Cout) if dzp is None else dzp[:, 1:1 + Lout].reshape(B * Lout, Cout)
                dcol = torch.empty(B * Lout, k * Cin, dtype=dy.dtype, device=dy.device)
                K.gemm(dz2, w_cl, dcol, B * Lout, k * Cin, Cout, a_kmajor=1, b_kmajor=0, lda=Cout, ldb=k * Cin, ldc=k * Cin, split_k=1)
                pzc = prev_z if prev_z is None else prev_z.contiguous()
                dx = K.col2im1d(dcol, pzc, B, Lin, Lout, Cin, k, stride, pad, L.ACT_GELU if prev_z is not None else 0)
        if ctx.needs_input_grad[1]:
            part = torch.empty(B, Cout, k * Cin, dtype=torch.float32, device=dy.device)
            wgs = B * ((Cout + 255) // 256) * ((k * Cin + 255) // 256)
            rem = wgs % 256
            sk = 2 if (wgs >= 256 and 0 < rem < 192 and Lout >= 2048) else 1
            dw = torch.empty(Cout, k * Cin, dtype=w_cl.dtype, device=dy.device)
            K.gemm(dz_rows, xp, part, Cout, k * Cin, Lout, a_kmajor=0, b_kmajor=0, lda=Cout, ldb=stride * Cin, ldc=k * Cin, batch0=B,
                   sa=(dz_bs, 0), sb=(xp.stride(0), 0), sc=(Cout * k * Cin, 0), a_off=dz_off, split_k=sk, k_len=ctx.nz_out, reduce_to=dw)
        if has_bias and ctx.needs_input_grad[2]:
            db = K.colsum(dz_rows.reshape(B * Lout, Cout) if dzp is None else dzp[:, 1:1 + Lout].reshape(B * Lout, Cout), w_cl.dtype)
        return dx, dw, db, None, None, None, None, None, None, None, None, None


def conv1d_cl(x, weight, bias, stride, pad=0, act=None, prev_z=None, grad_is_dz=False, nz_out=None, nz_in=None, unread_ok=False):
    Cout, Cin, k = weight.shape
    w_cl = weight.permute(0, 2, 1).reshape(Cout, k * Cin)
    if not w_cl.is_contiguous():
        w_cl = w_cl.contiguous()
    return _Conv1dCLFn.apply(x, w_cl, bias, k, stride, pad, _ACT[act], prev_z, bool(grad_is_dz), nz_out, nz_in, bool(unread_ok))


_POSCONV_DW_SPLIT = int(_os.environ.get("CST_POSCONV_DW_SPLIT", 1))
_POSCONV_WINDOW_CG, _POSCONV_WINDOW_KMAX = 48, 128


class _PosConvFn(torch.autograd.Function):

    @staticmethod
    def forward(ctx, x, weight, bias, groups, lens=None, grad_rows=None, grad_rows_host=None):
        B, T, C = x.shape
        k = weight.shape[2]
        cg = C // groups
        padl = k // 2
        Tp = T + k - 1 + (1 if k % 2 == 0 else 0)
        ml = None if lens is None else torch.clamp(lens.to(torch.int32) + padl, max=T).contiguous()
        window = (x.dtype == torch.bfloat16 and weight.dtype == x.dtype and cg == _POSCONV_WINDOW_CG and k <= _POSCONV_WINDOW_KMAX
                  and (bias is None or bias.dtype == x.dtype) and not _os.environ.get("CST_POSCONV_GEMM"))
        ctx.window = window
        if window:
            xc = x.contiguous()
            wg = weight.view(groups, cg, cg, k).permute(0, 1, 3, 2).contiguous()
            y, z = K.posconv_fwd(xc, wg, bias, groups, ml)
            ctx.save_for_backward(xc, weight, z)
            ctx.cfg = (B, T, C, k, groups, cg, padl, Tp)
            ctx.grad_rows, ctx.grad_rows_host = grad_rows, grad_rows_host
            return y
        xg = torch.empty(groups, B, Tp, cg, dtype=x.dtype, device=x.device)
        xg[:, :, :padl].zero_()
        xg[:, :, padl + T:].zero_()
        xg[:, :, padl:padl + T] = x.view(B, T, groups, cg).permute(2, 0, 1, 3)
        wg = weight.view(groups, cg, cg, k).permute(0, 1, 3, 2).contiguous()
        y = torch.empty(B, T, C, dtype=x.dtype, device=x.device)
        z = torch.empty_like(y)
        xc = x.contiguous()
        K.gemm(xg, wg, y, T, cg, k * cg, a_kmajor=1, b_kmajor=1, lda=cg, ldb=k * cg, ldc=C, batch0=B, batch1=groups,
               sa=(Tp * cg, B * Tp * cg), sb=(0, cg * k * cg), sc=(T * C, cg), bias=bias, sbias=(0, cg), act=L.ACT_GELU,
               aux_out=z, ld_aux_out=C, resid=xc, ld_resid=C, split_k=1, m_len=ml)
        ctx.save_for_backward(xg, weight, z)
        ctx.cfg = (B, T, C, k, groups, cg, padl, Tp)
        ctx.grad_rows, ctx.grad_rows_host = grad_rows, grad_rows_host
        return y

    @staticmethod
    def backward(ctx, dy):
        xg, weight, z = ctx.saved_tensors
# ... 344 lines not shown
```

chimera-st_amd/kernels.py:

```python
import ctypes
import os

import torch

from . import lib as L

_ws = {}
STATS = {}


def workspace(nbytes: int, device) -> torch.Tensor:
    key = (device.index, L.stream_ptr().value)
    t = _ws.get(key)
    if t is None or t.numel() < nbytes:
        t = torch.empty(max(nbytes, 1 << 20), dtype=torch.uint8, device=device)
        _ws[key] = t
    return t


class _Deferred:

    MAX_BYTES = 32 << 20

    def __init__(self):
# ... 19 lines not shown
    def flush(self):
        self.join()
        if self.items:
            reduce_multi(self.items)
            self.flushes += 1
            self.items, self.keep = [], []


DEFER = _Deferred()


def reduce_multi(items):
    lib = L.load()
    for at in range(0, len(items), 64):
        chunk = items[at:at + 64]
        arr = (L.ReduceItem * len(chunk))()
        for a, (src, dst, stride, Lr, P, dt, order) in zip(arr, chunk):
            a.src, a.dst, a.stride, a.L, a.P, a.dst_dtype, a.order = src, dst, stride, Lr, P, dt, order
        L.check(lib.cst_reduce_multi(arr, len(chunk), L.stream_ptr()), "cst_reduce_multi")


class deferred_reductions:

    def __init__(self, enabled=True):
        self.enabled = bool(enabled) and not os.environ.get("CST_NO_DEFER")

    def __enter__(self):
        if self.enabled:
            DEFER.on += 1
            DEFER.main = torch.cuda.current_stream()
            DEFER.poison = bool(os.environ.get("CST_DEFER_POISON"))
        return self

    def __exit__(self, *exc):
        if self.enabled:
            DEFER.on -= 1
            if DEFER.on == 0:
                DEFER.flush()
        return False


def side_gemm(big, reads, *args, **kw):
    if big or not DEFER.on or DEFER.main is None or not os.environ.get("CST_SIDE_STREAM") or torch.cuda.current_stream() != DEFER.main:
        return gemm(*args, **kw)
    if DEFER.side is None:
        DEFER.side = torch.cuda.Stream()
    side = DEFER.side
    side.wait_stream(DEFER.main)
    DEFER.side_used = True
    with torch.cuda.stream(side):
        out = gemm(*args, **kw)
    for t in reads:
        if t is not None:
            t.record_stream(side)
    STATS["side_gemm"] = STATS.get("side_gemm", 0) + 1
    return out


def _2d(t):
    assert t.dim() == 2 and t.stride(1) == 1, "expected a row-major 2-D tensor, got %s / %s" % (tuple(t.shape), t.stride())
    return t


def _stamps(live, extent, stat):
    if live is None:
        return None, 0
    assert live[0].numel() * 64 >= extent and live[0].dtype == torch.int32
    STATS[stat] = STATS.get(stat, 0) + 1
    return live[0].data_ptr(), live[1]


def _per_batch(v, batch0, stat):
    if v is None:
        return None
    assert v.dtype == torch.int32 and v.numel() == batch0 and v.is_contiguous()
    STATS[stat] = STATS.get(stat, 0) + 1
    return v.data_ptr()


def gemm(A, B, C, M, N, K, *, a_kmajor, b_kmajor, lda, ldb, ldc, bias=None, bias_mode=L.BIAS_COL, act=L.ACT_NONE,
         aux_out=None, ld_aux_out=0, dact=L.ACT_NONE, aux_in=None, ld_aux_in=0, resid=None, ld_resid=0, alpha=1.0,
         batch0=1, batch1=1, sa=(0, 0), sb=(0, 0), sc=(0, 0), sbias=(0, 0), a_seg=0, a_seg_stride=0, b_seg=0,
         b_seg_stride=0, split_k=-1, a_off=0, b_off=0, c_off=0, drop_p=0.0, drop_key=0, k_live=None, m_live=None, k_len=None, m_len=None,
         ws=None, colsum=None, defer=False, reduce_to=None):
    lib = L.load()
    d = L.GemmDesc()
    d.dtype = L.dtype_code(A.dtype)
    assert B.dtype == A.dtype, "A/B dtype mismatch"
    d.c_dtype = L.dtype_code(C.dtype)
    d.a_kmajor, d.b_kmajor = int(a_kmajor), int(b_kmajor)
    d.M, d.N, d.K = M, N, K
    es = A.element_size()
    d.A = A.data_ptr() + a_off * es
    d.lda, d.a_seg, d.a_seg_stride = lda, a_seg, a_seg_stride
    d.B = B.data_ptr() + b_off * es
    d.ldb, d.b_seg, d.b_seg_stride = ldb, b_seg, b_seg_stride
    d.C = C.data_ptr() + c_off * C.element_size()
    d.ldc = ldc
    if bias is not None:
        assert bias.dtype == A.dtype
        d.bias, d.bias_mode = bias.data_ptr(), bias_mode
    else:
        d.bias, d.bias_mode = None, L.BIAS_NONE
    d.sbias0, d.sbias1 = sbias
    d.act = act
    d.aux_out = None if aux_out is None else aux_out.data_ptr() + c_off * es
    d.ld_aux_out = ld_aux_out
    d.dact = dact
    d.aux_in = None if aux_in is None else aux_in.data_ptr() + c_off * es
    d.ld_aux_in = ld_aux_in
    d.resid = None if resid is None else resid.data_ptr() + c_off * es
    d.ld_resid = ld_resid
    d.alpha = alpha
    d.drop_p, d.drop_key = float(drop_p), int(drop_key) & 0xFFFFFFFF
    d.batch0, d.batch1 = batch0, batch1
    d.sa0, d.sa1 = sa
    d.sb0, d.sb1 = sb
    d.sc0, d.sc1 = sc
    d.split_k = split_k
    d.k_live, d.k_epoch = _stamps(k_live, K, "gemm_k_live")
    d.m_live, d.m_epoch = _stamps(m_live, M, "gemm_m_live")
    d.k_len = _per_batch(k_len, batch0, "gemm_k_len")
    d.m_len = _per_batch(m_len, batch0, "gemm_m_len")
    if colsum is not None:
        assert not a_kmajor and colsum.dtype == A.dtype and colsum.is_contiguous() and colsum.numel() == M * batch0 * batch1
        d.colsum = colsum.data_ptr()
    else:
        d.colsum = None
    d.defer_reduce = 0
    splits = 1
    need = lib.cst_gemm_workspace(ctypes.byref(d))
    nb = batch0 * batch1
    deferred = False
    if need > 0 and (reduce_to is not None or (defer and DEFER.on and nb == 1 and need <= DEFER.MAX_BYTES and ldc == N and N % 8 == 0)):
        splits = lib.cst_gemm_splits(ctypes.byref(d))
        if splits > 1:
            assert ws is None and bias is None and act == L.ACT_NONE and dact == L.ACT_NONE and resid is None and aux_out is None and alpha == 1.0
            ws = torch.empty(need, dtype=torch.uint8, device=A.device)
            d.defer_reduce = 1
            deferred = True
    if need > 0:
        if ws is None:
            ws = workspace(need, A.device)
        assert ws.dtype == torch.uint8 and ws.numel() >= need, "split-K scratch too small: %d < %d" % (ws.numel(), need)
        d.workspace, d.workspace_bytes = ws.data_ptr(), ws.numel()
    else:
        d.workspace, d.workspace_bytes = None, 0
    L.check(lib.cst_gemm(ctypes.byref(d), L.stream_ptr()), "cst_gemm")
    if reduce_to is not None:
        assert C.dtype == torch.float32 and sc == (M * N, 0) and ldc == N and reduce_to.numel() == M * N and reduce_to.is_contiguous() and colsum is None
        item = ((ws.data_ptr(), reduce_to, M * N, M * N, nb * splits, ws) if deferred else (C.data_ptr(), reduce_to, M * N, M * N, nb, C))
        if defer and DEFER.on:
            DEFER.push(*item)
        else:
            reduce_multi([(item[0], item[1].data_ptr(), item[2], item[3], item[4], L.dtype_code(reduce_to.dtype), 0)])
    elif deferred:
        DEFER.push(ws.data_ptr(), C, M * N, M * N, splits, ws)
        if colsum is not None:
            DEFER.push(ws.data_ptr() + 4 * splits * M * N, colsum, M, M, splits, ws)
    return C


_DW_FUSED = {}


def dw_colsum_is_fused(n_out, k_in, tokens, dtype):
    key = (n_out, k_in, tokens, dtype)
    r = _DW_FUSED.get(key)
    if r is None:
        d = L.GemmDesc()
        d.dtype = d.c_dtype = L.dtype_code(dtype)
        d.a_kmajor = d.b_kmajor = 0
        d.M, d.N, d.K = n_out, k_in, tokens
        d.batch0 = d.batch1 = 1
        d.split_k = -1
        d.colsum = 1
        r = _DW_FUSED[key] = bool(L.load().cst_gemm_colsum_is_fused(ctypes.byref(d)))
        if len(_DW_FUSED) > 4096:
            _DW_FUSED.clear()
    return r


def layernorm_fwd(x, res, gamma, beta, eps, want_sum=False):
    x = _2d(x)
    rows, cols = x.shape
    y = torch.empty_like(x)
    s = torch.empty_like(x) if (want_sum and res is not None) else None
    mean = torch.empty(rows, dtype=torch.float32, device=x.device)
    rstd = torch.empty(rows, dtype=torch.float32, device=x.device)
    L.check(L.load().cst_layernorm_fwd(L.ptr(x), L.ptr(res), L.ptr(gamma), L.ptr(beta), L.ptr(y), L.ptr(s), L.ptr(mean),
                                       L.ptr(rstd), rows, cols, eps, L.dtype_code(x.dtype), L.stream_ptr()), "cst_layernorm_fwd")
    return y, s, mean, rstd


_EPOCH = [0x3C6EF372]


def next_epoch():
    _EPOCH[0] = (_EPOCH[0] % 0xFFFFFFFE) + 1
    return _EPOCH[0]


def _two_stage(wbytes, outs, defer, launch):
    deferred = bool(defer) and DEFER.on > 0
    dev = outs[0].device
    ws = torch.empty(wbytes, dtype=torch.uint8, device=dev) if deferred else workspace(wbytes, dev)
    launch(ws, *[None if deferred else L.ptr(o) for o in outs])
    if deferred:
        n, cols = len(outs), outs[0].numel()
        for i, o in enumerate(outs):
            DEFER.push(ws.data_ptr() + 4 * cols * i, o, n * cols, cols, wbytes // (4 * n * cols), ws, order=1)


def layernorm_bwd(dy, s, gamma, mean, rstd, dres=None, grad_dtype=torch.float32, want_tiles=False, defer=False):
    dy, s = _2d(dy), _2d(s)
    rows, cols = s.shape
    lib = L.load()
    dx = torch.empty_like(s)
    dg = torch.empty(cols, dtype=grad_dtype, device=s.device)
    db = torch.empty(cols, dtype=grad_dtype, device=s.device)
    stamps, epoch = (torch.empty((rows + 63) // 64, dtype=torch.int32, device=s.device), next_epoch()) if want_tiles else (None, 0)

    def launch(ws, pg, pb):
        if want_tiles:
            L.check(lib.cst_layernorm_bwd_tiles(L.ptr(dy), L.ptr(s), L.ptr(gamma), L.ptr(mean), L.ptr(rstd), L.ptr(dres), L.ptr(dx), pg,
                                                pb, L.ptr(ws), rows, cols, L.dtype_code(s.dtype), L.dtype_code(grad_dtype),
                                                L.ptr(stamps), epoch, L.stream_ptr()), "cst_layernorm_bwd_tiles")
        else:
            L.check(lib.cst_layernorm_bwd(L.ptr(dy), L.ptr(s), L.ptr(gamma), L.ptr(mean), L.ptr(rstd), L.ptr(dres), L.ptr(dx), pg,
                                          pb, L.ptr(ws), rows, cols, L.dtype_code(s.dtype), L.dtype_code(grad_dtype), L.stream_ptr()),
                    "cst_layernorm_bwd")

    _two_stage(lib.cst_layernorm_bwd_workspace(rows, cols), (dg, db), defer, launch)
    return (dx, dg, db, (stamps, epoch)) if want_tiles else (dx, dg, db)


def _bhtd_strides(t, layout):
    assert t.stride(-1) == 1
    if layout == "bt":
        return t.stride(0), None, t.stride(1)
    return t.stride(1), None, t.stride(0)


def attn_desc(q, k, v, o, lse, H, D, kpm, causal, scale, layout_q="bt", layout_kv="bt", drop_p=0.0, drop_key=0, kv_len=None, seq=None):
    d = L.AttnDesc()
    d.dtype = L.dtype_code(q.dtype)
    if layout_q == "bt":
        B, Tq = q.shape[0], q.shape[1]
    else:
        Tq, B = q.shape[0], q.shape[1]
    Tk = k.shape[1] if layout_kv == "bt" else k.shape[0]
    if seq is not None:
        assert layout_q == "bt" and layout_kv == "bt" and B == 1 and kpm is None
        assert seq[0].dtype == torch.int32 and seq[0].is_contiguous()
        B, Tq, Tk = seq[0].numel() - 1, int(seq[1]), int(seq[1])
        d.seq_offsets = seq[0].data_ptr()
        STATS["attn_packed"] = STATS.get("attn_packed", 0) + 1
    else:
        d.seq_offsets = None
    d.B, d.H, d.Tq, d.Tk, d.D = B, H, Tq, Tk, D

    def st(t, lay):
        sb, _, stt = _bhtd_strides(t, lay)
        return sb, D, stt

# ... 760 lines not shown
```

chimera-st_amd/lib.py:

```python
import ctypes
import os

import torch

_HERE = os.path.dirname(os.path.abspath(__file__))
LIB_PATH = os.path.join(_HERE, "libcst_hip.so")
ABI_VERSION = 13

F32, BF16 = 0, 1
ACT_NONE, ACT_RELU, ACT_GELU = 0, 1, 2
BIAS_NONE, BIAS_COL, BIAS_ROW = 0, 1, 2
K_GEMM, K_ATTN_FWD, K_ATTN_BWD, K_LAYERNORM, K_CONV0, K_ELEMENTWISE, K_LOSS, K_OPTIM = range(8)
KERNEL_CLASSES = ["gemm", "attn_fwd", "attn_bwd", "layernorm", "conv0", "elementwise", "loss", "optim"]

c_i64, c_int, c_f, c_p = ctypes.c_int64, ctypes.c_int, ctypes.c_float, ctypes.c_void_p


class GemmDesc(ctypes.Structure):
    _fields_ = [
        ("dtype", c_int), ("c_dtype", c_int), ("a_kmajor", c_int), ("b_kmajor", c_int),
        ("M", c_i64), ("N", c_i64), ("K", c_i64),
        ("A", c_p), ("lda", c_i64), ("a_seg", c_i64), ("a_seg_stride", c_i64),
        ("B", c_p), ("ldb", c_i64), ("b_seg", c_i64), ("b_seg_stride", c_i64),
        ("C", c_p), ("ldc", c_i64),
        ("bias", c_p), ("bias_mode", c_int), ("sbias0", c_i64), ("sbias1", c_i64),
        ("act", c_int),
        ("aux_out", c_p), ("ld_aux_out", c_i64),
        ("dact", c_int),
        ("aux_in", c_p), ("ld_aux_in", c_i64),
        ("resid", c_p), ("ld_resid", c_i64),
        ("alpha", c_f),
        ("drop_p", c_f), ("drop_key", ctypes.c_uint32),
        ("batch0", c_i64), ("batch1", c_i64),
        ("sa0", c_i64), ("sa1", c_i64), ("sb0", c_i64), ("sb1", c_i64), ("sc0", c_i64), ("sc1", c_i64),
        ("split_k", c_int),
        ("workspace", c_p), ("workspace_bytes", c_i64),
        ("k_live", c_p), ("k_epoch", ctypes.c_uint32),
        ("m_live", c_p), ("m_epoch", ctypes.c_uint32),
        ("k_len", c_p),
        ("m_len", c_p),
        ("colsum", c_p),
        ("defer_reduce", c_int),
    ]


class ReduceItem(ctypes.Structure):
    _fields_ = [("src", c_p), ("dst", c_p), ("stride", c_i64), ("L", c_i64), ("P", ctypes.c_int32), ("dst_dtype", ctypes.c_int32),
                ("block0", ctypes.c_int32), ("order", ctypes.c_int32)]


class AttnDesc(ctypes.Structure):
    _fields_ = [
        ("dtype", c_int),
        ("B", c_i64), ("H", c_i64), ("Tq", c_i64), ("Tk", c_i64), ("D", c_i64),
        ("Q", c_p), ("q_sb", c_i64), ("q_sh", c_i64), ("q_st", c_i64),
        ("K", c_p), ("k_sb", c_i64), ("k_sh", c_i64), ("k_st", c_i64),
        ("V", c_p), ("v_sb", c_i64), ("v_sh", c_i64), ("v_st", c_i64),
        ("O", c_p), ("o_sb", c_i64), ("o_sh", c_i64), ("o_st", c_i64),
        ("lse", c_p),
        ("key_padding_mask", c_p), ("kpm_stride", c_i64),
        ("causal", c_int), ("scale", c_f),
        ("drop_p", c_f), ("drop_key", ctypes.c_uint32),
        ("dO", c_p), ("do_sb", c_i64), ("do_sh", c_i64), ("do_st", c_i64),
        ("dQ", c_p), ("dq_sb", c_i64), ("dq_sh", c_i64), ("dq_st", c_i64),
        ("dK", c_p), ("dk_sb", c_i64), ("dk_sh", c_i64), ("dk_st", c_i64),
        ("dV", c_p), ("dv_sb", c_i64), ("dv_sh", c_i64), ("dv_st", c_i64),
        ("delta", c_p),
        ("kv_len", c_p),
        ("q_flags", c_p),
        ("seq_offsets", c_p),
        ("kpm_bits", c_p),
        ("bwd_ws", c_p),
    ]


class BeamDesc(ctypes.Structure):
    _fields_ = [
        ("dtype", c_int),
        ("bsz", c_i64), ("beam", c_i64), ("vocab", c_i64), ("max_len", c_i64),
        ("pad", c_i64), ("unk", c_i64), ("eos", c_i64), ("min_len", c_i64),
        ("unk_penalty", c_f), ("len_penalty", c_f), ("temperature", c_f),
        ("normalize_scores", c_int),
        ("logits", c_p), ("ld_logits", c_i64),
        ("step", c_p),
        ("tokens", c_p), ("scores", c_p), ("anc", c_p),
        ("cands_to_ignore", c_p), ("finished", c_p), ("nfinal", c_p), ("num_remaining", c_p),
        ("fin_tokens", c_p), ("fin_pos", c_p), ("fin_score", c_p), ("fin_len", c_p),
        ("workspace", c_p),
        ("members", c_i64), ("logits_n", c_p * 7), ("lprobs_out", c_p),
        ("no_repeat_ngram", c_i64), ("prefix_tokens", c_p), ("prefix_len", c_i64),
        ("sampling", c_i64), ("sample_topk", c_i64), ("sample_topp", c_f), ("sample_key", c_p),
        ("diverse_groups", c_i64), ("diverse_strength", c_f), ("diverse_siblings", c_i64), ("sibling_rate", c_f),
        ("fin_anc", c_p),
    ]


class LmFusionDesc(ctypes.Structure):
    _fields_ = [("lm_logits", c_p), ("lm_weight", c_f), ("lprobs_out", c_p)]


class LexDesc(ctypes.Structure):
    _fields_ = [("representation", c_i64), ("constraints", c_p), ("width", c_i64), ("workspace", c_p)]


LEX_TBL_W, LEX_SW, LEX_NEXT_MAX, LEX_WIDTH_MAX = 136, 44, 16, 65


def lex_states(workspace, bsz, beam):
    words = workspace.view(torch.int32)
    return words[bsz * LEX_TBL_W:bsz * LEX_TBL_W + 2 * bsz * beam * LEX_SW].view(2, bsz * beam, LEX_SW)


class FbankDesc(ctypes.Structure):
    _fields_ = [
        ("B", c_i64), ("S", c_i64), ("T", c_i64),
        ("wave", c_p), ("n_samples", c_p), ("out", c_p), ("n_frames", c_p),
        ("utterance_cmvn", c_int), ("norm_means", c_int), ("norm_vars", c_int),
        ("global_mean", c_p), ("global_std", c_p),
        ("global_first", c_int),
        ("specaugment", c_int),
        ("n_fmask", c_int), ("n_tmask", c_int),
        ("fmask", c_p), ("tmask", c_p),
        ("mask_mean", c_int), ("mask_value", c_f),
        ("workspace", c_p), ("workspace_bytes", c_i64),
    ]


SYMBOLS = [
    ("cst_last_error", ctypes.c_char_p, []),
    ("cst_version", c_int, []),
    ("cst_device_arch_ok", c_int, []),
    ("cst_prof_enable", None, [c_int]),
    ("cst_prof_query", c_i64, [c_int, ctypes.POINTER(ctypes.c_double), ctypes.POINTER(ctypes.c_double), ctypes.POINTER(ctypes.c_double)]),
    ("cst_layernorm_fwd", c_int, [c_p, c_p, c_p, c_p, c_p, c_p, c_p, c_p, c_i64, c_i64, c_f, c_int, c_p]),
    ("cst_layernorm_bwd_workspace", c_i64, [c_i64, c_i64]),
    ("cst_layernorm_bwd", c_int, [c_p, c_p, c_p, c_p, c_p, c_p, c_p, c_p, c_p, c_p, c_i64, c_i64, c_int, c_int, c_p]),
    ("cst_layernorm_bwd_tiles", c_int, [c_p, c_p, c_p, c_p, c_p, c_p, c_p, c_p, c_p, c_p, c_i64, c_i64, c_int, c_int, c_p, ctypes.c_uint32, c_p]),
    ("cst_gemm_workspace", c_i64, [ctypes.POINTER(GemmDesc)]),
    ("cst_gemm_colsum_is_fused", c_int, [ctypes.POINTER(GemmDesc)]),
    ("cst_gemm_splits", c_int, [ctypes.POINTER(GemmDesc)]),
    ("cst_gemm_route", c_int, [ctypes.POINTER(GemmDesc), ctypes.c_char_p, c_i64]),
    ("cst_reduce_multi", c_int, [ctypes.POINTER(ReduceItem), c_int, c_p]),
    ("cst_gemm", c_int, [ctypes.POINTER(GemmDesc), c_p]),
    ("cst_posconv_fwd", c_int, [c_p, c_p, c_p, c_p, c_p, c_p, c_i64, c_i64, c_i64, c_i64, c_i64, c_p]),
    ("cst_posconv_dx", c_int, [c_p, c_p, c_p, c_p, c_p, c_i64, c_i64, c_i64, c_i64, c_i64, c_p]),
    ("cst_posconv_dw", c_int, [c_p, c_p, c_p, c_p, c_p, ctypes.c_uint32, c_i64, c_i64, c_i64, c_i64, c_i64, c_p]),
    ("cst_prof_dump", c_i64, [c_int, ctypes.c_char_p, c_i64]),
    ("cst_gemm_reserve_cus", c_int, [c_int]),
    ("cst_transpose2d", c_int, [c_p, c_p, c_i64, c_i64, c_int, c_p]),
    ("cst_transpose2d_multi", c_int, [c_p, c_int, c_i64, c_int, c_p]),
    ("cst_weight_norm_workspace", c_i64, [c_i64, c_i64]),
    ("cst_weight_norm_fwd", c_int, [c_p, c_p, c_p, c_p, c_p, c_i64, c_i64, c_int, c_p]),
    ("cst_weight_norm_bwd", c_int, [c_p, c_p, c_p, c_p, c_p, c_p, c_p, c_i64, c_i64, c_int, c_p]),
    ("cst_attn_bwd_workspace", c_i64, [ctypes.POINTER(AttnDesc)]),
    ("cst_attn_fwd", c_int, [ctypes.POINTER(AttnDesc), c_p]),
    ("cst_attn_bwd", c_int, [ctypes.POINTER(AttnDesc), c_p]),
    ("cst_conv0_fwd_workspace", c_i64, [c_i64, c_i64, c_int, c_int]),
    ("cst_conv0_gn_gelu_fwd", c_int, [c_p, c_p, c_p, c_p, c_p, c_p, c_p, c_p, c_p, c_p, c_i64, c_i64, c_i64, c_int, c_int, c_f, c_int, c_p]),
    ("cst_conv0_bwd_workspace", c_i64, [c_i64, c_i64, c_i64, c_int, c_int]),
    ("cst_conv0_gn_gelu_bwd", c_int, [c_p, c_p, c_p, c_p, c_p, c_p, c_p, c_p, c_p, c_p, c_p, c_p, c_p, c_i64, c_i64, c_i64, c_int, c_int, c_int, c_p]),
    ("cst_conv0_ln_gelu_fwd", c_int, [c_p, c_p, c_p, c_p, c_p, c_p, c_p, c_p, c_p, c_i64, c_i64, c_i64, c_int, c_int, c_f, c_int, c_p]),
    ("cst_conv0_ln_bwd_workspace", c_i64, [c_i64, c_i64, c_i64, c_int, c_int]),
    ("cst_conv0_ln_gelu_bwd", c_int, [c_p, c_p, c_p, c_p, c_p, c_p, c_p, c_p, c_p, c_p, c_p, c_p, c_p, c_p, c_i64, c_i64, c_i64, c_int, c_int, c_int, c_p]),
    ("cst_ln_gelu_fwd", c_int, [c_p, c_p, c_p, c_p, c_p, c_p, c_p, c_i64, c_i64, c_i64, c_f, c_int, c_p]),
    ("cst_ln_gelu_bwd_workspace", c_i64, [c_i64, c_i64]),
    ("cst_ln_gelu_bwd", c_int, [c_p, c_p, c_p, c_p, c_p, c_p, c_p, c_i64, c_p, c_p, c_p, c_p, c_p, c_i64, c_i64, c_i64, c_int, c_p]),
    ("cst_glu_fwd", c_int, [c_p, c_p, c_i64, c_i64, c_int, c_p]),
    ("cst_glu_bwd", c_int, [c_p, c_p, c_p, c_i64, c_i64, c_int, c_p]),
    ("cst_act_bwd", c_int, [c_p, c_p, c_p, c_i64, c_int, c_int, c_p]),
    ("cst_act_fwd", c_int, [c_p, c_p, c_i64, c_int, c_int, c_p]),
    ("cst_colsum", c_int, [c_p, c_i64, c_p, c_i64, c_i64, c_int, c_p]),
    ("cst_colsum_workspace", c_i64, [c_i64, c_i64]),
    ("cst_colsum_typed", c_int, [c_p, c_i64, c_p, c_p, c_i64, c_i64, c_int, c_int, c_p]),
    ("cst_colsum_typed_live", c_int, [c_p, c_i64, c_p, c_p, c_i64, c_i64, c_int, c_int, c_p, ctypes.c_uint32, c_p]),
    ("cst_col2im1d", c_int, [c_p, c_p, c_p, c_i64, c_i64, c_i64, c_i64, c_int, c_int, c_int, c_int, c_int, c_p]),
    ("cst_mask_rows", c_int, [c_p, c_p, c_p, c_i64, c_i64, c_int, c_p]),
    ("cst_dropout", c_int, [c_p, c_p, c_i64, c_f, ctypes.c_uint32, c_int, c_p]),
    ("cst_rows_pack", c_int, [c_p, c_p, c_p, c_i64, c_i64, c_i64, c_int, c_int, c_p]),
    ("cst_rows_unpack", c_int, [c_p, c_p, c_p, c_i64, c_i64, c_i64, c_int, c_int, c_p]),
    ("cst_dec_linear", c_int, [c_p, c_p, c_p, c_p, c_p, c_i64, c_i64, c_i64, c_i64, c_i64, c_i64, c_int, c_p, c_i64, c_int, c_p]),
    ("cst_dec_ln_linear", c_int, [c_p, c_p, c_p, c_p, c_f, c_p, c_p, c_i64, c_i64, c_i64, c_i64, c_i64, c_i64, c_int, c_p, c_i64, c_int, c_p]),
    ("cst_dropout_colsum", c_int, [c_p, c_p, c_p, c_p, c_i64, c_i64, c_int, c_int, c_f, ctypes.c_uint32, c_p, ctypes.c_uint32, c_p]),
    ("cst_conv_row_limits", c_int, [c_p, c_p, c_p, c_int, c_i64, c_p, c_i64, c_int, c_p]),
    ("cst_dropout_scale", c_int, [c_p, c_p, c_i64, c_f, c_f, ctypes.c_uint32, c_int, c_p]),
    ("cst_embed_pos_fwd", c_int, [c_p, c_p, c_p, c_p, c_p, c_f, c_i64, c_p, c_i64, c_i64, c_i64, c_i64, c_i64, c_f, ctypes.c_uint32, c_int, c_p]),
    ("cst_embed_bwd", c_int, [c_p, c_p, c_p, c_f, c_i64, c_i64, c_i64, c_i64, c_f, ctypes.c_uint32, c_int, c_int, c_p]),
    ("cst_ls_ce_fwd", c_int, [c_p, c_p, c_p, c_p, c_p, c_i64, c_i64, c_f, c_i64, c_int, c_p]),
    ("cst_ls_ce_bwd", c_int, [c_p, c_p, c_p, c_p, c_p, c_i64, c_i64, c_f, c_i64, c_int, c_p]),
    ("cst_score_tokens", c_int, [c_p, ctypes.POINTER(c_p), c_i64, c_i64, c_p, c_i64, c_p, c_p, c_p, c_i64, c_i64, c_i64, c_int, c_p]),
    ("cst_ctc_fwd", c_int, [c_p, c_i64, c_i64, c_p, c_i64, c_p, c_p, c_i64, c_int, c_p, c_p, c_p, c_p, c_p, c_p, c_i64, c_i64, c_i64, c_int, c_p]),
    ("cst_ctc_bwd", c_int, [c_p, c_i64, c_i64, c_p, c_i64, c_p, c_p, c_i64, c_int, c_p, c_p, c_p, c_p, c_p, c_p, c_i64, c_i64, c_i64, c_i64, c_i64,
                            c_int, c_p]),
    ("cst_ctc_greedy", c_int, [c_p, c_i64, c_i64, c_p, c_i64, c_p, c_p, c_p, c_i64, c_i64, c_i64, c_int, c_p]),
    ("cst_w2v_negatives", c_int, [ctypes.c_uint32, c_i64, c_i64, c_i64, c_i64, c_p, c_p]),
    ("cst_infonce_fwd", c_int, [c_p, c_p, c_p, c_f, c_p, c_p, c_p, c_p, c_p, c_p, c_p, c_p, c_i64, c_i64, c_i64, c_int, c_p]),
    ("cst_infonce_bwd_x", c_int, [c_p, c_p, c_p, c_f, c_p, c_p, c_p, c_p, c_p, c_p, c_i64, c_i64, c_i64, c_int, c_p]),
    ("cst_infonce_bwd_y", c_int, [c_p, c_p, c_p, c_p, c_p, c_p, c_p, c_p, c_i64, c_i64, c_i64, c_int, c_p]),
    ("cst_gumbel_vq_workspace", c_i64, [c_i64, c_i64, c_i64]),
    ("cst_gumbel_vq_fwd", c_int, [c_p, c_p, c_p, ctypes.c_uint32, c_int, c_p, c_p, c_p, c_p, c_p, c_p, c_p, c_i64, c_i64, c_i64, c_i64, c_int, c_p]),
    ("cst_gumbel_vq_bwd", c_int, [c_p, c_p, ctypes.c_uint32, c_f, c_p, c_p, c_p, c_p, c_p, c_i64, c_i64, c_i64, c_int, c_p]),
    ("cst_contrastive_fwd", c_int, [c_p, c_p, c_p, c_p, c_p, c_p, c_p, c_i64, c_i64, c_i64, c_f, c_int, c_p]),
    ("cst_contrastive_bwd", c_int, [c_p, c_p, c_p, c_p, c_p, c_p, c_p, c_p, c_i64, c_i64, c_i64, c_f, c_int, c_p]),
    ("cst_sumsq_workspace", c_i64, []),
    ("cst_sumsq", c_int, [c_p, c_i64, c_p, c_p, c_int, c_p]),
    ("cst_adam_step", c_int, [c_p, c_p, c_p, c_p, c_p, c_i64, c_f, c_f, c_f, c_f, c_f, c_i64, c_p, c_int, c_int, c_p]),
    ("cst_beam_workspace", c_i64, [c_i64, c_i64]),
    ("cst_beam_init", c_int, [ctypes.POINTER(BeamDesc), c_p]),
    ("cst_beam_step", c_int, [ctypes.POINTER(BeamDesc), c_p]),
    ("cst_beam_step_lm", c_int, [ctypes.POINTER(BeamDesc), ctypes.POINTER(LmFusionDesc), c_p]),
    ("cst_lex_workspace", c_i64, [c_i64, c_i64, c_i64]),
    ("cst_lex_init", c_int, [ctypes.POINTER(BeamDesc), ctypes.POINTER(LexDesc), c_p]),
    ("cst_beam_step_lex", c_int, [ctypes.POINTER(BeamDesc), ctypes.POINTER(LmFusionDesc), ctypes.POINTER(LexDesc), c_p]),
    ("cst_dec_embed", c_int, [c_p, c_p, c_p, c_p, c_f, c_i64, c_p, c_i64, c_i64, c_i64, c_i64, c_int, c_p]),
    ("cst_dec_self_attn", c_int, [c_p, c_p, c_p, c_p, c_p, c_p, c_i64, c_i64, c_i64, c_i64, c_f, c_int, c_p]),
    ("cst_batch_by_size", c_i64, [c_p, c_i64, c_i64, c_i64, ctypes.c_int32, c_p]),
    ("cst_wav_info", c_int, [ctypes.c_char_p, c_p, c_p, c_p, c_p]),
    ("cst_wav_read_f32", c_i64, [ctypes.c_char_p, c_i64, c_i64, c_p, c_i64]),
    ("cst_edit_distance", c_i64, [c_p, c_i64, c_p, c_i64]),
    ("cst_dec_cross_attn", c_int, [c_p, c_p, c_p, c_p, c_p, c_p, c_i64, c_i64, c_i64, c_i64, c_i64, c_i64, c_f, c_int, c_p]),
    ("cst_fbank_workspace_bytes", c_i64, [c_i64, c_i64]),
    ("cst_fbank", c_int, [ctypes.POINTER(FbankDesc), c_p]),
    ("cst_dec_ln_q_cross_attn", c_int, [c_p, c_i64, c_p, c_p, c_p, c_f, c_p, c_p, c_p, c_p, c_p, c_i64, c_i64, c_i64, c_i64, c_i64, c_i64, c_f, c_int, c_p]),
    ("cst_attn_avg_probs", c_int, [c_p, c_i64, c_p, c_i64, c_i64, c_i64, c_p, c_p, c_i64, c_p, c_i64, c_i64, c_i64, c_i64, c_i64, c_i64, c_f, c_f,
                                   c_int, c_int, c_p]),
    ("cst_collate_pairs", c_int, [c_p, c_p, c_int, c_p, c_p, c_i64, c_p, c_i64, c_i64, c_i64, c_i64, c_i64, c_int, c_int, c_p, c_p]),
    ("cst_token_block_slices", c_i64, [c_p, c_i64, c_int, c_i64, c_i64, c_p, c_i64]),
    ("cst_token_block_index", c_int, [c_p, c_i64, c_p, c_i64, c_p]),
    ("cst_collate_blocks", c_int, [c_p, c_int, c_p, c_i64, c_p, c_i64, c_i64, c_i64, c_i64, c_p, c_p]),
]

_lib = None


# ... 78 lines not shown
```

include/cst.h:

```cpp
#ifndef CST_H
#define CST_H

#include <stdint.h>

#ifdef __cplusplus
extern "C" {
#endif

#define CST_ABI_VERSION 13

typedef enum { CST_F32 = 0, CST_BF16 = 1 } cst_dtype;

typedef enum {
  CST_OK = 0,
  CST_ERR_BAD_ARG = -1,
  CST_ERR_LAUNCH = -2,
  CST_ERR_WORKSPACE = -3,
  CST_ERR_UNSUPPORTED = -4
} cst_status;

typedef void* cst_stream;

const char* cst_last_error(void);
int cst_version(void);
int cst_device_arch_ok(void);

typedef enum {
  CST_K_GEMM = 0, CST_K_ATTN_FWD, CST_K_ATTN_BWD, CST_K_LAYERNORM, CST_K_CONV0, CST_K_ELEMENTWISE,
  CST_K_LOSS, CST_K_OPTIM, CST_K_NUM
} cst_kernel_class;
void cst_prof_enable(int on);
int64_t cst_prof_query(int kernel_class, double* total_ms, double* flops, double* bytes);
int64_t cst_prof_dump(int kernel_class, char* buf, int64_t cap);

int cst_layernorm_fwd(const void* x, const void* res, const void* gamma, const void* beta,
                      void* y, void* sum_out, float* mean, float* rstd,
                      int64_t rows, int64_t cols, float eps, int dtype, cst_stream stream);
int64_t cst_layernorm_bwd_workspace(int64_t rows, int64_t cols);
int cst_layernorm_bwd(const void* dy, const void* s, const void* gamma, const float* mean,
                      const float* rstd, const void* dres, void* dx, void* dgamma, void* dbeta,
                      void* workspace, int64_t rows, int64_t cols, int dtype, int grad_dtype, cst_stream stream);
int cst_layernorm_bwd_tiles(const void* dy, const void* s, const void* gamma, const float* mean,
                            const float* rstd, const void* dres, void* dx, void* dgamma, void* dbeta,
                            void* workspace, int64_t rows, int64_t cols, int dtype, int grad_dtype,
                            uint32_t* tile_live, uint32_t epoch, cst_stream stream);

typedef enum { CST_ACT_NONE = 0, CST_ACT_RELU = 1, CST_ACT_GELU = 2 } cst_act;
typedef enum { CST_BIAS_NONE = 0, CST_BIAS_COL = 1, CST_BIAS_ROW = 2 } cst_bias_mode;

typedef struct {
  int dtype;
  int c_dtype;
  int a_kmajor, b_kmajor;
  int64_t M, N, K;
  const void* A; int64_t lda, a_seg, a_seg_stride;
  const void* B; int64_t ldb, b_seg, b_seg_stride;
  void* C; int64_t ldc;
  const void* bias; int bias_mode;
  int64_t sbias0, sbias1;
  int act;
  void* aux_out; int64_t ld_aux_out;
  int dact;
  const void* aux_in; int64_t ld_aux_in;
  const void* resid; int64_t ld_resid;
  float alpha;
  float drop_p; uint32_t drop_key;
  int64_t batch0, batch1;
  int64_t sa0, sa1, sb0, sb1, sc0, sc1;
  int split_k;
  void* workspace; int64_t workspace_bytes;
  const uint32_t* k_live; uint32_t k_epoch;
  const uint32_t* m_live; uint32_t m_epoch;
  const int32_t* k_len;
  const int32_t* m_len;
  void* colsum;
  int defer_reduce;
} cst_gemm_desc;

int64_t cst_gemm_workspace(const cst_gemm_desc* d);
int cst_gemm_colsum_is_fused(const cst_gemm_desc* d);
int cst_gemm_splits(const cst_gemm_desc* d);
int cst_gemm_route(const cst_gemm_desc* d, char* out, int64_t out_bytes);
int cst_gemm_reserve_cus(int n);
int cst_gemm(const cst_gemm_desc* d, cst_stream stream);

int cst_posconv_fwd(const void* x, const void* w, const void* bias, void* y, void* z, const int32_t* m_len, int64_t B, int64_t T,
                    int64_t C, int64_t groups, int64_t k, cst_stream stream);
int cst_posconv_dx(const void* dz, const void* wflip, const void* dy, void* dx, const int32_t* m_len, int64_t B, int64_t T,
                   int64_t C, int64_t groups, int64_t k, cst_stream stream);
int cst_posconv_dw(const void* dz, const void* x, void* dw, void* db, const uint32_t* k_live, uint32_t k_epoch, int64_t B,
                   int64_t T, int64_t C, int64_t groups, int64_t k, cst_stream stream);

typedef struct {
  int dtype;
  int64_t B, H, Tq, Tk, D;
  const void* Q; int64_t q_sb, q_sh, q_st;
  const void* K; int64_t k_sb, k_sh, k_st;
  const void* V; int64_t v_sb, v_sh, v_st;
  void* O; int64_t o_sb, o_sh, o_st;
  float* lse;
  const uint8_t* key_padding_mask; int64_t kpm_stride;
  int causal;
  float scale;
  float drop_p; uint32_t drop_key;
  const void* dO; int64_t do_sb, do_sh, do_st;
  void* dQ; int64_t dq_sb, dq_sh, dq_st;
  void* dK; int64_t dk_sb, dk_sh, dk_st;
  void* dV; int64_t dv_sb, dv_sh, dv_st;
  float* delta;
  const int32_t* kv_len;
  uint8_t* q_flags;
  const int32_t* seq_offsets;
  const uint64_t* kpm_bits;
  void* bwd_ws;
} cst_attn_desc;

int64_t cst_attn_bwd_workspace(const cst_attn_desc* d);
int cst_attn_fwd(const cst_attn_desc* d, cst_stream stream);
int cst_attn_bwd(const cst_attn_desc* d, cst_stream stream);

int cst_conv_row_limits(const int32_t* nz_last, const int32_t* k, const int32_t* stride, int L, int64_t S, int32_t* out, int64_t B,
                        int smax, cst_stream stream);
int64_t cst_conv0_fwd_workspace(int64_t B, int64_t S, int k, int stride);
int cst_conv0_gn_gelu_fwd(const float* wav, const void* w, const void* gamma, const void* beta,
                          void* y, float* mean, float* rstd, float* gram, float* workspace, const int32_t* frame_limit, int64_t B,
                          int64_t S, int64_t C, int k, int stride, float eps, int dtype, cst_stream stream);
int64_t cst_conv0_bwd_workspace(int64_t B, int64_t S, int64_t C, int k, int stride);
int cst_conv0_gn_gelu_bwd(const void* dy, const float* wav, const void* w, const void* gamma,
                          const void* beta, const float* mean, const float* rstd, const float* gram,
                          float* dw, float* dgamma, float* dbeta, float* workspace, const int32_t* frame_limit,
                          int64_t B, int64_t S, int64_t C, int k, int stride, int dtype,
                          cst_stream stream);

int cst_conv0_ln_gelu_fwd(const float* wav, const void* w, const void* bias, const void* gamma, const void* beta, void* y,
                          float* mean, float* rstd, const int32_t* frame_limit, int64_t B, int64_t S, int64_t C, int k,
                          int stride, float eps, int dtype, cst_stream stream);
int64_t cst_conv0_ln_bwd_workspace(int64_t B, int64_t S, int64_t C, int k, int stride);
int cst_conv0_ln_gelu_bwd(const void* dy, const float* wav, const void* w, const void* bias, const void* gamma, const void* beta,
                          const float* mean, const float* rstd, float* dw, float* dbias, float* dgamma, float* dbeta,
                          float* workspace, const int32_t* frame_limit, int64_t B, int64_t S, int64_t C, int k, int stride,
                          int dtype, cst_stream stream);
int cst_ln_gelu_fwd(const void* u, const void* gamma, const void* beta, void* y, float* mean, float* rstd,
                    const int32_t* row_limit, int64_t B, int64_t L, int64_t C, float eps, int dtype, cst_stream stream);
int64_t cst_ln_gelu_bwd_workspace(int64_t rows, int64_t C);
int cst_ln_gelu_bwd(const void* dy, const void* u, const void* gamma, const void* beta, const float* mean, const float* rstd,
                    void* du, int64_t du_batch_stride, float* dgamma, float* dbeta, float* dcolsum, float* workspace,
                    const int32_t* row_limit, int64_t B, int64_t L, int64_t C, int dtype, cst_stream stream);

int cst_glu_fwd(const void* z, void* y, int64_t rows, int64_t C, int dtype, cst_stream stream);
int cst_glu_bwd(const void* dy, const void* z, void* dz, int64_t rows, int64_t C, int dtype, cst_stream stream);
int cst_act_bwd(const void* dy, const void* z, void* dx, int64_t n, int act, int dtype, cst_stream stream);
int cst_act_fwd(const void* x, void* y, int64_t n, int act, int dtype, cst_stream stream);
int cst_colsum(const void* x, int64_t ldx, float* out, int64_t rows, int64_t cols, int dtype, cst_stream stream);
int cst_dropout_colsum(const void* x, void* xd, void* out, void* workspace, int64_t rows, int64_t cols, int dtype, int out_dtype,
                       float p, uint32_t key, const uint32_t* row_live, uint32_t epoch, cst_stream stream);
int64_t cst_colsum_workspace(int64_t rows, int64_t cols);
int cst_colsum_typed(const void* x, int64_t ldx, void* out, void* workspace, int64_t rows, int64_t cols, int dtype, int out_dtype,
                     cst_stream stream);
int cst_colsum_typed_live(const void* x, int64_t ldx, void* out, void* workspace, int64_t rows, int64_t cols, int dtype,
                          int out_dtype, const uint32_t* row_live, uint32_t epoch, cst_stream stream);
int cst_col2im1d(const void* dcol, const void* z, void* dx, int64_t B, int64_t Lin, int64_t Lout,
                 int64_t C, int k, int stride, int pad, int dact, int dtype, cst_stream stream);
int64_t cst_weight_norm_workspace(int64_t R, int64_t C);
int cst_weight_norm_fwd(const void* v, const void* g, void* w, float* norm, void* workspace, int64_t R, int64_t C, int dtype, cst_stream stream);
int cst_weight_norm_bwd(const void* v, const void* g, const void* dw, const float* norm, void* dv, void* dg, void* workspace, int64_t R,
                        int64_t C, int dtype, cst_stream stream);
int cst_transpose2d(const void* src, void* dst, int64_t R, int64_t C, int dtype, cst_stream stream);
typedef struct cst_transpose_item {
  const void* src; void* dst;
  int64_t R, C;
  int64_t tile0;
} cst_transpose_item;
int cst_transpose2d_multi(const cst_transpose_item* items_dev, int n, int64_t total_tiles, int dtype, cst_stream stream);
#define CST_REDUCE_MAX_ITEMS 64
typedef struct cst_reduce_item {
  const float* src; void* dst;
  int64_t stride, L;
  int32_t P, dst_dtype, block0, order;
} cst_reduce_item;
int cst_reduce_multi(const cst_reduce_item* items, int n, cst_stream stream);
int cst_mask_rows(const void* x, const uint8_t* mask, void* y, int64_t rows, int64_t cols, int dtype, cst_stream stream);

int cst_rows_pack(const void* src, const int32_t* seq_off, void* dst, int64_t B, int64_t T, int64_t C, int tail_sum, int dtype,
                  cst_stream stream);
int cst_rows_unpack(const void* src, const int32_t* seq_off, void* dst, int64_t B, int64_t T, int64_t C, int tail_broadcast, int dtype,
                    cst_stream stream);

int cst_dropout(const void* x, void* y, int64_t n, float p, uint32_t key, int dtype, cst_stream stream);
int cst_dropout_scale(const void* x, void* y, int64_t n, float alpha, float p, uint32_t key, int dtype, cst_stream stream);

int cst_embed_pos_fwd(const int64_t* tokens, const uint8_t* pad_mask, const void* embed, const void* x, const float* pos_table,
                      float scale, int64_t pad_idx, void* out, int64_t B, int64_t T, int64_t C, int64_t V, int64_t pos_rows,
                      float drop_p, uint32_t drop_key, int dtype, cst_stream stream);
int cst_embed_bwd(const void* dy, const int64_t* tokens, void* dE, float scale, int64_t pad_idx, int64_t n, int64_t C, int64_t V,
                  float drop_p, uint32_t drop_key, int dtype, int grad_dtype, cst_stream stream);

int cst_ls_ce_fwd(const void* logits, const int64_t* target, float* out2, float* lse, float* row_ws,
                  int64_t rows, int64_t V, float eps, int64_t pad_idx, int dtype, cst_stream stream);
int cst_ls_ce_bwd(const void* logits, const int64_t* target, const float* lse, const float* gscale,
                  void* dlogits, int64_t rows, int64_t V, float eps, int64_t pad_idx, int dtype,
                  cst_stream stream);

int cst_score_tokens(const void* logits, const void* const* logits_n, int64_t members, int64_t ld, const int64_t* target, int64_t pad,
                     float* pos, float* score, int32_t* len, int64_t B, int64_t T, int64_t V, int dtype, cst_stream stream);

int cst_ctc_fwd(const void* logits, int64_t stride_t, int64_t stride_b, const int64_t* targets, int64_t Lmax, const int64_t* target_len,
                const int64_t* input_len, int64_t blank, int zero_infinity, float* nll, float* loss, float* lse, float* emit, float* alpha,
                float* beta, int64_t T, int64_t B, int64_t V, int dtype, cst_stream stream);
int cst_ctc_bwd(const void* logits, int64_t stride_t, int64_t stride_b, const int64_t* targets, int64_t Lmax, const int64_t* target_len,
                const int64_t* input_len, int64_t blank, int zero_infinity, const float* nll, const float* lse, const float* alpha,
                const float* beta, const float* gscale, void* dlogits, int64_t dstride_t, int64_t dstride_b, int64_t T, int64_t B,
                int64_t V, int dtype, cst_stream stream);
int cst_ctc_greedy(const void* logits, int64_t stride_t, int64_t stride_b, const int64_t* input_len, int64_t blank, int32_t* argmax_ws,
                   int32_t* ids, int32_t* counts, int64_t T, int64_t B, int64_t V, int dtype, cst_stream stream);

int cst_w2v_negatives(uint32_t key, int64_t B, int64_t M, int64_t K, int64_t Kx, int32_t* out, cst_stream stream);
int cst_infonce_fwd(const void* x, const void* y, const int32_t* idx, float inv_temp, float* nll, float* loss, int32_t* counters,
                    float* lse, float* nx, float* ny, int32_t* flags, float* logits_dbg, int64_t N, int64_t KP, int64_t D, int dtype,
                    cst_stream stream);
int cst_infonce_bwd_x(const void* x, const void* y, const int32_t* idx, float inv_temp, const float* lse, const float* nx,
                      const float* ny, const float* gscale, void* dx, float* pairs, int64_t N, int64_t KP, int64_t D, int dtype,
                      cst_stream stream);
int cst_infonce_bwd_y(const void* x, const void* y, const int64_t* perm, const int32_t* offs, const float* pairs, const float* nx,
                      const float* ny, void* dy, int64_t N, int64_t KP, int64_t D, int dtype, cst_stream stream);

int64_t cst_gumbel_vq_workspace(int64_t N, int64_t G, int64_t V);
int cst_gumbel_vq_fwd(const void* logits, const void* vars, const float* noise, uint32_t key, int training, void* q, int32_t* idx,
                      void* onehot, float* avg_probs, float* stats, float* exph, void* workspace, int64_t N, int64_t G, int64_t V, int64_t d,
                      int dtype, cst_stream stream);
int cst_gumbel_vq_bwd(const void* logits, const float* noise, uint32_t key, float inv_tau, const void* gy, const float* avg_probs,
                      const float* exph, const float* dppl, void* dl, int64_t N, int64_t G, int64_t V, int dtype, cst_stream stream);

int cst_contrastive_fwd(const void* a, const void* t, float* loss, float* loss_rows, float* sim, float* na, float* nt,
                        int64_t B, int64_t M, int64_t C, float temp, int dtype, cst_stream stream);
int cst_contrastive_bwd(const void* a, const void* t, const float* sim, const float* na, const float* nt,
                        const float* gscale, void* da, void* dt, int64_t B, int64_t M, int64_t C, float temp,
                        int dtype, cst_stream stream);

int64_t cst_sumsq_workspace(void);
int cst_sumsq(const void* x, int64_t n, float* out, float* workspace, int dtype, cst_stream stream);
int cst_adam_step(float* master, float* exp_avg, float* exp_avg_sq, const void* grad, void* model_param,
                  int64_t n, float lr, float beta1, float beta2, float eps, float weight_decay,
                  int64_t step, const float* grad_scale, int grad_dtype, int param_dtype,
                  cst_stream stream);

typedef struct {
  int dtype;
  int64_t bsz, beam, vocab, max_len;
  int64_t pad, unk, eos, min_len;
  float unk_penalty, len_penalty, temperature;
  int normalize_scores;
  const void* logits; int64_t ld_logits;
  int32_t* step;
  int64_t* tokens; float* scores; int32_t* anc;
  uint8_t* cands_to_ignore; uint8_t* finished; int32_t* nfinal; int32_t* num_remaining;
  int64_t* fin_tokens; float* fin_pos; float* fin_score; int32_t* fin_len;
// ... 98 lines not shown
```

Baseline: 515.8.

## Merge per-residue strided conv input-gradient GEMMs into one column-blocked GEMM

The strided 1D conv backward-data pass used to launch one GEMM per stride residue. It now builds a combined, transposed and zero-padded weight matrix with a new kernel and runs a single GEMM. Each column block of that GEMM has its own K start offset, row limit and per-batch length. This cuts kernel launches and fills the GPU better for the small per-residue problems, at the cost of an extra weight reshuffle kernel, zero-padded taps in the K loop, and more per-tile branching in the GEMM kernels.

New measurement: 505.2. 2.0% lower.

```diff
diff --git a/chimera-st_amd/csrc/elementwise.hip b/chimera-st_amd/csrc/elementwise.hip
--- a/chimera-st_amd/csrc/elementwise.hip
+++ b/chimera-st_amd/csrc/elementwise.hip
@@ -637,6 +637,43 @@
 }
 
 namespace {
+template <typename T>
+__global__ __launch_bounds__(256) void conv_dx_weights_kernel(const T* __restrict__ w, T* __restrict__ out, int Cout, int Cin, int k, int s, int nmax) {
+  __shared__ T tile[64][65];
+  const int r = (int)blockIdx.z / nmax, g = (int)blockIdx.z % nmax;
+  const int j = r + s * (nmax - 1 - g);
+  const int ci0 = blockIdx.x * 64, co0 = blockIdx.y * 64;
+  const int tx = threadIdx.x & 63, ty = threadIdx.x >> 6;
+  if (j < k) {
+    for (int i = ty; i < 64; i += 4) {
+      const int co = co0 + i, ci = ci0 + tx;
+      if (co < Cout && ci < Cin) tile[i][tx] = w[(int64_t)co * k * Cin + (int64_t)j * Cin + ci];
+    }
+  }
+  __syncthreads();
+  for (int i = ty; i < 64; i += 4) {
+    const int ci = ci0 + i, co = co0 + tx;
+    if (ci < Cin && co < Cout) out[((int64_t)r * Cin + ci) * nmax * Cout + (int64_t)g * Cout + co] = j < k ? tile[tx][i] : T(0.0f);
+  }
+}
+}
+
+extern "C" int cst_conv_dx_weights(const void* w_cl, void* out, int64_t Cout, int64_t Cin, int64_t k, int64_t stride, int dtype, cst_stream stream) {
+  CST_REQUIRE(w_cl && out && Cout > 0 && Cin > 0 && k > 0 && stride > 0 && stride <= 4, "cst_conv_dx_weights: bad arguments");
+  CST_REQUIRE(dtype == CST_F32 || dtype == CST_BF16, "cst_conv_dx_weights: bad dtype");
+  const int64_t nmax = (k + stride - 1) / stride;
+  CST_REQUIRE(Cout * k * Cin < (1ll << 31) && stride * nmax < 65536 && (Cout + 63) / 64 < 65536, "cst_conv_dx_weights: too large");
+  hipStream_t s = (hipStream_t)stream;
+  CstProfScope prof(CST_K_ELEMENTWISE, s, 0.0, (double)(Cout * k * Cin + stride * Cin * nmax * Cout) * cst_dtype_size(dtype));
+  const dim3 grid((unsigned)((Cin + 63) / 64), (unsigned)((Cout + 63) / 64), (unsigned)(stride * nmax));
+  if (dtype == CST_BF16)
+    hipLaunchKernelGGL(conv_dx_weights_kernel<bf16_t>, grid, dim3(256), 0, s, (const bf16_t*)w_cl, (bf16_t*)out, (int)Cout, (int)Cin, (int)k, (int)stride, (int)nmax);
+  else
+    hipLaunchKernelGGL(conv_dx_weights_kernel<float>, grid, dim3(256), 0, s, (const float*)w_cl, (float*)out, (int)Cout, (int)Cin, (int)k, (int)stride, (int)nmax);
+  return cst_check_launch("cst_conv_dx_weights");
+}
+
+namespace {
 struct ReduceTable { cst_reduce_item it[CST_REDUCE_MAX_ITEMS]; int n; };
 
 __global__ __launch_bounds__(1024) void reduce_multi_kernel(ReduceTable t) {
diff --git a/chimera-st_amd/csrc/gemm.hip b/chimera-st_amd/csrc/gemm.hip
--- a/chimera-st_amd/csrc/gemm.hip
+++ b/chimera-st_amd/csrc/gemm.hip
@@ -82,8 +82,16 @@
     ktiles = live < ktiles ? live : ktiles;
   }
   const int per = (ktiles + p.splits - 1) / p.splits;
-  const int kt0 = split * per;
+  int kt0 = split * per;
   const int kt1 = (kt0 + per < ktiles) ? kt0 + per : ktiles;
+  int64_t mlim = p.M;
+  const int32_t* mlen = p.m_len;
+  if (p.col_block > 0) {
+    const int blk = col_block_of(n0, p.col_block);
+    kt0 = (blk == 0 ? p.k_begin[0] : blk == 1 ? p.k_begin[1] : blk == 2 ? p.k_begin[2] : p.k_begin[3]) / BK;
+    mlim = blk == 0 ? p.m_rows[0] : blk == 1 ? p.m_rows[1] : blk == 2 ? p.m_rows[2] : p.m_rows[3];
+    mlen = blk == 0 ? p.m_len_blk[0] : blk == 1 ? p.m_len_blk[1] : blk == 2 ? p.m_len_blk[2] : p.m_len_blk[3];
+  }
 
   u32x4 ra[NVA], rb[NVB];
   const T* pa[NVA];
@@ -241,10 +249,11 @@
     for (int t = t0; t < t1; ++t) live |= ml[t] == p.m_epoch;
     if (!live) nk = 0;
   }
-  if (p.m_len) {
+  if (mlen) {
     typedef const __attribute__((address_space(4))) int32_t* cptr_t;
-    if (m0 >= (int64_t)((cptr_t)p.m_len)[b0]) nk = 0;
-  }
+    if (m0 >= (int64_t)((cptr_t)mlen)[b0]) nk = 0;
+  }
+  if (m0 >= mlim) nk = 0;
   int pos = kt0;
   auto fetch = [&](int kt) {
     const int d = kt - pos;
@@ -335,7 +344,7 @@
       const int v = tid + NTHREADS * it;
       const int rl = v / VPR, cl = (v % VPR) * 8;
       const int64_t row = m0 + 64 * ps + rl, col = n0 + cl;
-      if (row >= p.M || col >= p.N) continue;
+      if (row >= mlim || col >= p.N) continue;
       float x[8];
       {
         const f32x4 a = *reinterpret_cast<const f32x4*>(stage + rl * LDC + cl);
@@ -836,6 +845,7 @@
   int stages;
   int splits;
   Colsum colsum;
+  bool colblocks;
 };
 
 struct TileDims { int bm, bn, nt; };
@@ -889,6 +899,7 @@
 
 GemmRoute gemm_route(const cst_gemm_desc* d, const GemmParams& p, const GemmSwitches& sw) {
   GemmRoute r;
+  r.colblocks = true;
   r.bf16 = d->dtype == CST_BF16;
   r.ak = d->a_kmajor != 0;
   r.bk = d->b_kmajor != 0;
@@ -899,7 +910,19 @@
   const bool large = use_large(d, r.seg, r.splits);
   const int64_t nbatch = d->batch0 * d->batch1;
   r.colsum = !d->colsum ? Colsum::None : (mm && !d->a_seg && !d->b_seg && !large) ? Colsum::Fused : Colsum::Separate;
-  auto take = [&r](Family f, Tile t, int stages = 2) { r.family = f; r.tile = t; r.stages = stages; return r; };
+  auto take = [&r, d](Family f, Tile t, int stages = 2) {
+    r.family = f; r.tile = t; r.stages = stages;
+    if (d->col_block > 0) {
+      if (f == Family::Dma) { r.family = Family::Reg; r.tile = t == Tile::Large ? Tile::Large : Tile::Small; }
+      const int bn = kTileDims[(int)r.tile].bn, bk = r.bf16 ? 64 : 32;
+      bool ok = r.family != Family::FourWave && r.tile != Tile::Unknown && !r.seg && r.splits == 1 && !d->colsum && !d->k_live && !d->m_live && !d->k_len &&
+                bn > 0 && d->col_block % bn == 0 && d->N <= 4 * d->col_block;
+      const int64_t nblk = ok ? cst_ceil_div(d->N, d->col_block) : 0;
+      for (int64_t b = 0; b < nblk; ++b) ok = ok && d->k_begin[b] >= 0 && d->k_begin[b] <= d->K && d->k_begin[b] % bk == 0;
+      r.colblocks = ok;
+    }
+    return r;
+  };
 
   if (!sw.no_narrow && !r.seg && !large && kk && d->N <= 64 && d->M > 256) return take(Family::Dma, Tile::NarrowN);
   if (!sw.no_narrow && !r.seg && !large && mm && d->M <= 64 && d->N > 256) return take(Family::Reg, Tile::NarrowM);
@@ -976,6 +999,14 @@
   CST_REQUIRE(d->drop_p >= 0.0f && d->drop_p < 1.0f, "cst_gemm: drop_p must be in [0, 1)");
   CST_REQUIRE(d->drop_p == 0.0f || d->batch0 * d->batch1 == 1, "cst_gemm: fused dropout needs an unbatched problem");
   CST_REQUIRE(!d->colsum || (!d->a_kmajor && !d->a_seg), "cst_gemm: colsum needs an mn-major, unsegmented A");
+  CST_REQUIRE(d->col_block >= 0, "cst_gemm: col_block must be >= 0");
+  if (d->col_block > 0) {
+    CST_REQUIRE(d->N <= 4 * d->col_block && d->M < (1ll << 31) && d->K < (1ll << 31) && d->col_block < (1ll << 31), "cst_gemm: at most 4 column blocks (N=%lld col_block=%lld)",
+                (long long)d->N, (long long)d->col_block);
+    for (int64_t b = 0; b < cst_ceil_div(d->N, d->col_block); ++b)
+      CST_REQUIRE(d->k_begin[b] >= 0 && d->k_begin[b] <= d->K && d->m_rows[b] >= 1 && d->m_rows[b] <= d->M,
+                  "cst_gemm: column block %d: k_begin=%lld outside [0, K] or m_rows=%lld outside [1, M]", (int)b, (long long)d->k_begin[b], (long long)d->m_rows[b]);
+  }
   return CST_OK;
 }
 
@@ -1024,6 +1055,19 @@
   p.ws = nullptr;
   p.colsum = nullptr;
   p.colsum_ws = nullptr;
+  p.col_block = 0;
+  for (int b = 0; b < 4; ++b) { p.k_begin[b] = 0; p.m_rows[b] = 0; p.m_len_blk[b] = nullptr; }
+  if (d->col_block > 0 && d->col_block < (1ll << 31)) {
+    p.col_block = (int)d->col_block;
+    const int64_t nblk = cst_ceil_div(d->N, d->col_block);
+    for (int b = 0; b < 4; ++b) {
+      const bool used = b < nblk;
+      p.k_begin[b] = used ? (int)d->k_begin[b] : 0;
+      p.m_rows[b] = (int)(used ? d->m_rows[b] : d->M);
+      p.m_len_blk[b] = (used && !sw.no_klive) ? d->m_len_blk[b] : nullptr;
+    }
+    p.m_len = nullptr;
+  }
   return p;
 }
 
@@ -1038,6 +1082,11 @@
 int take_route(const cst_gemm_desc* d, const GemmSwitches& sw, GemmParams& p, GemmRoute& r) {
   r = gemm_route(d, p, sw);
   const int64_t nbatch = d->batch0 * d->batch1;
+  if (!r.colblocks) {
+    cst_set_error("cst_gemm: column blocks (col_block=%lld) are not supported for this launch: col_block / k_begin do not fit the tiles of its kernel, "
+                  "or the kernel does not implement them (cst_gemm_colblocks_supported)", (long long)d->col_block);
+    return CST_ERR_UNSUPPORTED;
+  }
   CST_REQUIRE(r.colsum != Colsum::Separate || (nbatch == 1 && d->M % 8 == 0 && d->lda % 8 == 0),
               "cst_gemm: colsum of this configuration runs as a separate column sum: unbatched, M and lda multiples of 8");
   CST_REQUIRE(cst_ceil_div(d->M, 128) * cst_ceil_div(d->N, 128) < (1ll << 31) && nbatch * r.splits < 65536, "cst_gemm: grid too large");
@@ -1214,6 +1263,8 @@
 
 extern "C" int64_t cst_gemm_workspace(const cst_gemm_desc* d) { return route_workspace(d, query_route(d)); }
 
+extern "C" int cst_gemm_colblocks_supported(const cst_gemm_desc* d) { return d && d->col_block > 0 && query_route(d).colblocks ? 1 : 0; }
+
 extern "C" int cst_gemm_route(const cst_gemm_desc* d, char* out, int64_t out_bytes) {
   if (out && out_bytes > 0) out[0] = 0;
   int rc = validate(d);
diff --git a/chimera-st_amd/csrc/gemm8p.hip b/chimera-st_amd/csrc/gemm8p.hip
--- a/chimera-st_amd/csrc/gemm8p.hip
+++ b/chimera-st_amd/csrc/gemm8p.hip
@@ -135,7 +135,7 @@
     const T* B = (const T*)p.B + b0 * p.sb0 + b1 * p.sb1;
     cofs = b0 * p.sc0 + b1 * p.sc1;
     bofs = b0 * p.sbias0 + b1 * p.sbias1;
-    const int kt0 = split * per;
+    int kt0 = split * per;
     const int kt1 = (kt0 + per < ktiles) ? kt0 + per : ktiles;
     nt = kt1 > kt0 ? kt1 - kt0 : 0;
     if (kp->m_live) {
@@ -148,9 +148,19 @@
       for (int i = 0; i < 4; ++i) live |= (i < 2 || !hf) && (t0 + i < tn) && ml[t0 + i < tn ? t0 + i : t0] == ep;
       if (!live) nt = 0;
     }
+    typedef const __attribute__((address_space(4))) int32_t* iptr_t;
     if (kp->m_len) {
-      typedef const __attribute__((address_space(4))) int32_t* iptr_t;
       if (m0 >= (int64_t)((iptr_t)kp->m_len)[b0]) nt = 0;
+    }
+    mrem = (int)(p.M - m0 < BM ? p.M - m0 : BM);
+    if (kp->col_block > 0) {
+      const int blk = col_block_of(n0, kp->col_block);
+      kt0 = kp->k_begin[blk] >> 6;
+      nt = ktiles - kt0;
+      const int64_t left = (int64_t)kp->m_rows[blk] - m0;
+      mrem = (int)(left < BM ? left : BM);
+      iptr_t mlen = (iptr_t)kp->m_len_blk[blk];
+      if (mlen && m0 >= (int64_t)mlen[b0]) nt = 0;
     }
     krem0 = (int)p.K - kt0 * BK;
     const T* abase = AK ? A + m0 * p.lda + (int64_t)kt0 * BK : A + (int64_t)kt0 * BK * p.lda + m0;
@@ -165,7 +175,6 @@
     }
     lda2 = (unsigned)(p.lda * 2);
     ldb2 = (unsigned)(p.ldb * 2);
-    mrem = (int)(p.M - m0 < BM ? p.M - m0 : BM);
     if (hf && mrem > 128) mrem = 128;
     if (mrem <= 0) { mrem = 0; nt = 0; }
     nrem = (int)(p.N - n0 < BN ? p.N - n0 : BN);
@@ -386,6 +395,7 @@
     q.aux_out = kp->aux_out; q.ld_aux_out = kp->ld_aux_out; q.dact = kp->dact; q.aux_in = kp->aux_in; q.ld_aux_in = kp->ld_aux_in;
     q.resid = kp->resid; q.ld_resid = kp->ld_resid; q.alpha = kp->alpha; q.splits = kp->splits; q.ws = kp->ws;
     q.c_f32 = kp->c_f32; q.vec_epi = kp->vec_epi; q.drop_thr = kp->drop_thr; q.drop_key = kp->drop_key; q.drop_scale = kp->drop_scale; q.drop_row0 = kp->drop_row0;
+    if (kp->col_block > 0) q.M = kp->m_rows[col_block_of(e_n0, kp->col_block)];
     if (fast_epi && e_nt == 0 && q.bias_mode == CST_BIAS_NONE && !q.resid) {
       if (has_next) claim_land();
       const u32x4 z4 = {0u, 0u, 0u, 0u};
@@ -709,8 +719,9 @@
     for (int sft = 0; sft < 16; ++sft)
       if ((1 << sft) == p.group_m) p.group_shift = sft;
     const int gfull = p.tiles_m / p.group_m;
-    p.gperm_full = (p.m_len && gfull >= 16) ? gfull : 0;
-    p.mrot = (p.m_len && p.gperm_full == 0 && ntl >= 2) ? (int)(ntl / 8 > 0 ? ntl / 8 : 1) : 0;
+    const bool row_limits = p.m_len || (p.col_block > 0 && (p.m_len_blk[0] || p.m_len_blk[1] || p.m_len_blk[2] || p.m_len_blk[3]));
+    p.gperm_full = (row_limits && gfull >= 16) ? gfull : 0;
+    p.mrot = (row_limits && p.gperm_full == 0 && ntl >= 2) ? (int)(ntl / 8 > 0 ? ntl / 8 : 1) : 0;
     p.gperm_q = gfull / 8;
     p.gperm_r = gfull % 8;
     p.magic_gq = p.gperm_q > 0 ? ((1ull << 40) / (unsigned long long)p.gperm_q) + 1ull : 0ull;
diff --git a/chimera-st_amd/csrc/gemm_common.h b/chimera-st_amd/csrc/gemm_common.h
--- a/chimera-st_amd/csrc/gemm_common.h
+++ b/chimera-st_amd/csrc/gemm_common.h
@@ -42,7 +42,12 @@
   const uint32_t* k_live; uint32_t k_epoch;
   void* colsum;
   float* colsum_ws;
+  int col_block;
+  int k_begin[4], m_rows[4];
+  const int32_t* m_len_blk[4];
 };
+
+__device__ __forceinline__ int col_block_of(int64_t n0, int cb) { return (int)(n0 >= cb) + (int)(n0 >= 2 * (int64_t)cb) + (int)(n0 >= 3 * (int64_t)cb); }
 
 __device__ __forceinline__ int64_t segaddr(int64_t c, int64_t seg, int64_t seg_stride) {
   return seg ? (c / seg) * seg_stride + (c % seg) : c;
diff --git a/chimera-st_amd/functional.py b/chimera-st_amd/functional.py
--- a/chimera-st_amd/functional.py
+++ b/chimera-st_amd/functional.py
@@ -806,7 +806,22 @@
                 pz = prev_z if prev_z is None or dx_padded else prev_z.contiguous()
                 pz_base = _padded_base(prev_z, Lin, Cin) if dx_padded else pz
                 w3 = w_cl.view(Cout, k, Cin)
-                for r in range(stride):
+                dact = L.ACT_GELU if prev_z is not None else L.ACT_NONE
+                nmax = (k + stride - 1) // stride
+                taps_n = [len(range(r, k, stride)) for r in range(stride)]
+                U_all = [(Lin - r + stride - 1) // stride for r in range(stride)]
+                k_begin = [(nmax - n) * Cout for n in taps_n]
+                merged = (1 < stride <= 4 and min(taps_n) >= 1 and min(U_all) >= 1 and not _os.environ.get("CST_CONV_DX_PER_RESIDUE")
+                          and K.gemm_colblocks_supported(dy.dtype, U_all[0], stride * Cin, nmax * Cout, B, Cout, nmax * Cout, Cin, k_begin,
+                                                         prev_z is not None))
+                if merged:
+                    wm = K.conv_dx_weights(w_cl, Cout, Cin, k, stride)
+                    mlb = [ctx.nz_in[r] for r in range(stride)] if ctx.nz_in is not None else None
+                    K.gemm(dzp, wm, dx_full, U_all[0], stride * Cin, nmax * Cout, a_kmajor=1, b_kmajor=1, lda=Cout, ldb=nmax * Cout,
+                           ldc=stride * Cin, batch0=B, sa=((Lout + 2) * Cout, 0), sc=(rows * Cin, 0), a_off=(2 - nmax) * Cout,
+                           c_off=Cin if dx_padded else 0, dact=dact, aux_in=pz_base, ld_aux_in=stride * Cin, split_k=1,
+                           col_blocks=(Cin, k_begin, U_all, mlb))
+                for r in (() if merged else range(stride)):
                     taps = list(range(r, k, stride))
                     n = len(taps)
                     U = (Lin - r + stride - 1) // stride
diff --git a/chimera-st_amd/kernels.py b/chimera-st_amd/kernels.py
--- a/chimera-st_amd/kernels.py
+++ b/chimera-st_amd/kernels.py
@@ -125,7 +125,7 @@
          aux_out=None, ld_aux_out=0, dact=L.ACT_NONE, aux_in=None, ld_aux_in=0, resid=None, ld_resid=0, alpha=1.0,
          batch0=1, batch1=1, sa=(0, 0), sb=(0, 0), sc=(0, 0), sbias=(0, 0), a_seg=0, a_seg_stride=0, b_seg=0,
          b_seg_stride=0, split_k=-1, a_off=0, b_off=0, c_off=0, drop_p=0.0, drop_key=0, k_live=None, m_live=None, k_len=None, m_len=None,
-         ws=None, colsum=None, defer=False, reduce_to=None):
+         ws=None, colsum=None, defer=False, reduce_to=None, col_blocks=None):
     lib = L.load()
     d = L.GemmDesc()
     d.dtype = L.dtype_code(A.dtype)
@@ -165,6 +165,13 @@
     d.m_live, d.m_epoch = _stamps(m_live, M, "gemm_m_live")
     d.k_len = _per_batch(k_len, batch0, "gemm_k_len")
     d.m_len = _per_batch(m_len, batch0, "gemm_m_len")
+    if col_blocks is not None:
+        cb, kb, mr, mlb = col_blocks
+        assert m_len is None and len(kb) == len(mr) == (N + cb - 1) // cb <= 4
+        d.col_block = cb
+        for i in range(len(kb)):
+            d.k_begin[i], d.m_rows[i] = kb[i], mr[i]
+            d.m_len_blk[i] = None if mlb is None else _per_batch(mlb[i], batch0, "gemm_m_len")
     if colsum is not None:
         assert not a_kmajor and colsum.dtype == A.dtype and colsum.is_contiguous() and colsum.numel() == M * batch0 * batch1
         d.colsum = colsum.data_ptr()
@@ -224,6 +231,39 @@
     return r
 
 
+_COLBLOCKS = {}
+
+
+def gemm_colblocks_supported(dtype, M, N, K, batch0, lda, ldb, col_block, k_begin, dact):
+    key = (dtype, M, N, K, batch0, lda, ldb, col_block, tuple(k_begin), bool(dact))
+    r = _COLBLOCKS.get(key)
+    if r is None:
+        d = L.GemmDesc()
+        d.dtype = d.c_dtype = L.dtype_code(dtype)
+        d.a_kmajor = d.b_kmajor = 1
+        d.M, d.N, d.K = M, N, K
+        d.lda, d.ldb = lda, ldb
+        d.batch0, d.batch1 = batch0, 1
+        d.split_k = 1
+        d.dact = L.ACT_GELU if dact else L.ACT_NONE
+        d.aux_in = 16 if dact else None
+        d.col_block = col_block
+        for i, kb in enumerate(k_begin):
+            d.k_begin[i], d.m_rows[i] = kb, M
+        r = _COLBLOCKS[key] = bool(L.load().cst_gemm_colblocks_supported(ctypes.byref(d)))
+        if len(_COLBLOCKS) > 4096:
+            _COLBLOCKS.clear()
+    return r
+
+
+def conv_dx_weights(w_cl, Cout, Cin, k, stride):
+    assert w_cl.is_contiguous() and w_cl.shape == (Cout, k * Cin)
+    nmax = (k + stride - 1) // stride
+    out = torch.empty(stride * Cin, nmax * Cout, dtype=w_cl.dtype, device=w_cl.device)
+    L.check(L.load().cst_conv_dx_weights(L.ptr(w_cl), L.ptr(out), Cout, Cin, k, stride, L.dtype_code(w_cl.dtype), L.stream_ptr()), "cst_conv_dx_weights")
+    return out
+
+
 def layernorm_fwd(x, res, gamma, beta, eps, want_sum=False):
     x = _2d(x)
     rows, cols = x.shape
diff --git a/chimera-st_amd/lib.py b/chimera-st_amd/lib.py
--- a/chimera-st_amd/lib.py
+++ b/chimera-st_amd/lib.py
@@ -41,6 +41,7 @@
         ("m_len", c_p),
         ("colsum", c_p),
         ("defer_reduce", c_int),
+        ("col_block", c_i64), ("k_begin", c_i64 * 4), ("m_rows", c_i64 * 4), ("m_len_blk", c_p * 4),
     ]
 
 
@@ -140,6 +141,7 @@
     ("cst_gemm_colsum_is_fused", c_int, [ctypes.POINTER(GemmDesc)]),
     ("cst_gemm_splits", c_int, [ctypes.POINTER(GemmDesc)]),
     ("cst_gemm_route", c_int, [ctypes.POINTER(GemmDesc), ctypes.c_char_p, c_i64]),
+    ("cst_gemm_colblocks_supported", c_int, [ctypes.POINTER(GemmDesc)]),
     ("cst_reduce_multi", c_int, [ctypes.POINTER(ReduceItem), c_int, c_p]),
     ("cst_gemm", c_int, [ctypes.POINTER(GemmDesc), c_p]),
     ("cst_posconv_fwd", c_int, [c_p, c_p, c_p, c_p, c_p, c_p, c_i64, c_i64, c_i64, c_i64, c_i64, c_p]),
@@ -149,6 +151,7 @@
     ("cst_gemm_reserve_cus", c_int, [c_int]),
     ("cst_transpose2d", c_int, [c_p, c_p, c_i64, c_i64, c_int, c_p]),
     ("cst_transpose2d_multi", c_int, [c_p, c_int, c_i64, c_int, c_p]),
+    ("cst_conv_dx_weights", c_int, [c_p, c_p, c_i64, c_i64, c_i64, c_i64, c_int, c_p]),
     ("cst_weight_norm_workspace", c_i64, [c_i64, c_i64]),
     ("cst_weight_norm_fwd", c_int, [c_p, c_p, c_p, c_p, c_p, c_i64, c_i64, c_int, c_p]),
     ("cst_weight_norm_bwd", c_int, [c_p, c_p, c_p, c_p, c_p, c_p, c_p, c_i64, c_i64, c_int, c_p]),
diff --git a/include/cst.h b/include/cst.h
--- a/include/cst.h
+++ b/include/cst.h
@@ -75,12 +75,17 @@
   const int32_t* m_len;
   void* colsum;
   int defer_reduce;
+  int64_t col_block;
+  int64_t k_begin[4];
+  int64_t m_rows[4];
+  const int32_t* m_len_blk[4];
 } cst_gemm_desc;
 
 int64_t cst_gemm_workspace(const cst_gemm_desc* d);
 int cst_gemm_colsum_is_fused(const cst_gemm_desc* d);
 int cst_gemm_splits(const cst_gemm_desc* d);
 int cst_gemm_route(const cst_gemm_desc* d, char* out, int64_t out_bytes);
+int cst_gemm_colblocks_supported(const cst_gemm_desc* d);
 int cst_gemm_reserve_cus(int n);
 int cst_gemm(const cst_gemm_desc* d, cst_stream stream);
 
@@ -172,6 +177,7 @@
   int64_t tile0;
 } cst_transpose_item;
 int cst_transpose2d_multi(const cst_transpose_item* items_dev, int n, int64_t total_tiles, int dtype, cst_stream stream);
+int cst_conv_dx_weights(const void* w_cl, void* out, int64_t Cout, int64_t Cin, int64_t k, int64_t stride, int dtype, cst_stream stream);
 #define CST_REDUCE_MAX_ITEMS 64
 typedef struct cst_reduce_item {
   const float* src; void* dst;
```
